# TAMUparametric/PPOPT

Hardware: NVIDIA B200
Metric: candidate active sets/sec (higher is better)
Workload: dtype f64

## Files before the change

### include/ppgpu.h

```cpp
#ifndef PPGPU_H
#define PPGPU_H

#include <stddef.h>
#include <stdint.h>

#ifdef __cplusplus
extern "C" {
#endif

typedef struct ppgpu_program ppgpu_program;
typedef void* ppgpu_stream;

typedef struct {
    int32_t n;
    int32_t t;
    int32_t m;
    int32_t q;
    int32_t n_eq;
    int32_t is_qp;
} ppgpu_dims;

typedef struct {
    int32_t words;
    int32_t n_ineq;
    int32_t region_rows;
    int32_t use_gram;
    int32_t max_depth;
    int32_t sm_count;
    int32_t lp_columns;
    int32_t reserved;
} ppgpu_info;

#define PPGPU_NUM_COUNTERS 24

const char* ppgpu_last_error(void);
int ppgpu_version(void);

int ppgpu_program_create(const ppgpu_dims* dims, const double* h_A, const double* h_b, const double* h_F,
                         const double* h_A_t, const double* h_b_t, const double* h_Q, const double* h_c,
                         const double* h_H, int device, ppgpu_program** out);
int ppgpu_program_destroy(ppgpu_program* prog);
int ppgpu_program_info(const ppgpu_program* prog, ppgpu_info* out);

#define PPGPU_OPT_K2W_MIN 0
int ppgpu_set_option(ppgpu_program* prog, int32_t option, int64_t value);

int ppgpu_root_level(ppgpu_program* prog, uint64_t* d_masks, int64_t* h_count, ppgpu_stream stream);

int ppgpu_level_eval(ppgpu_program* prog, const uint64_t* d_masks, int64_t n, int32_t k_act, uint8_t* d_status,
                     int32_t stages, ppgpu_stream stream);

#define PPGPU_WITNESS_SLOTS 2
int ppgpu_level_eval_w(ppgpu_program* prog, const uint64_t* d_masks, int64_t n, int32_t k_act, uint8_t* d_status,
                       int32_t stages, uint64_t* d_witness, const uint64_t* d_parent_feas, int64_t parent_nf,
                       const void* d_parent_ws, const uint64_t* d_parent_wit, ppgpu_stream stream);

size_t ppgpu_scan_workspace_bytes(int64_t n);
int ppgpu_level_select(ppgpu_program* prog, const uint8_t* d_status, int64_t n, uint8_t bits, uint8_t value,
                       int64_t* d_idx_out, int64_t* h_count, void* d_ws, size_t ws_bytes, ppgpu_stream stream);

int ppgpu_regions_emit(ppgpu_program* prog, const uint64_t* d_masks, const int64_t* d_sel, int64_t n_sel,
                       int32_t k_act, double* d_laws, double* d_rows, int32_t* d_flags, double* d_info,
                       uint8_t* d_status, ppgpu_stream stream);

int ppgpu_children_count(ppgpu_program* prog, const uint64_t* d_masks, const int64_t* d_feas_idx, int64_t nf,
                         int32_t k_act, uint64_t* d_feas_masks, uint64_t* d_survive, int64_t* d_offsets,
                         int64_t* h_total, void* d_ws, size_t ws_bytes, ppgpu_stream stream);
int ppgpu_children_prepare(ppgpu_program* prog, const uint64_t* d_masks, const int64_t* d_feas_idx, int64_t nf,
                           uint64_t* d_feas_masks, void* d_ws, size_t ws_bytes, ppgpu_stream stream);
int ppgpu_children_count_range(ppgpu_program* prog, const uint64_t* d_feas_masks, int64_t nf, int32_t k_act,
                               uint64_t* d_survive, int64_t* d_counts, int64_t p_lo, int64_t p_hi, void* d_ws,
                               size_t ws_bytes, ppgpu_stream stream);
int ppgpu_children_scan(ppgpu_program* prog, int64_t* d_counts_to_offsets, int64_t nf, int64_t* h_total, void* d_ws,
                        size_t ws_bytes, ppgpu_stream stream);
int ppgpu_children_write(ppgpu_program* prog, const uint64_t* d_feas_masks, const uint64_t* d_survive,
                         const int64_t* d_offsets, int64_t nf, uint64_t* d_children, ppgpu_stream stream);

int ppgpu_locate_points(const double* d_theta, int64_t n_points, int32_t t, const double* d_rows, const int64_t* d_row_off,
                        int64_t n_regions, const double* d_laws, int32_t n_x, int32_t use_tol, double tol, int32_t overlap,
                        const double* d_Q, const double* d_H, const double* d_c, int32_t* d_region, double* d_x,
                        ppgpu_stream stream);

int ppgpu_solve_theta_batch(ppgpu_program* prog, const double* d_theta, int64_t n_points, uint8_t* d_status, double* d_x,
                            double* d_dual, uint64_t* d_active, int32_t* d_iters, ppgpu_stream stream);

int ppgpu_solve_theta_lp_batch(ppgpu_program* prog, const double* d_theta, int64_t n_points, uint8_t* d_status, double* d_x,
                               double* d_dual, uint64_t* d_active, int32_t* d_iters, ppgpu_stream stream);

int ppgpu_chebyshev_batch(const double* d_rows, const int64_t* d_row_off, int64_t n_polytopes, int32_t t, int32_t max_rows,
                          double* d_radius, int32_t* d_code, ppgpu_stream stream);

int ppgpu_counters(ppgpu_program* prog, uint64_t* h_out, int32_t reset, ppgpu_stream stream);

int64_t ppgpu_launch_count(const ppgpu_program* prog);

#define PPGPU_NUM_FAMILIES 10
int ppgpu_profile_enable(ppgpu_program* prog, int32_t on);
int ppgpu_profile_read(ppgpu_program* prog, double* h_ms, int64_t* h_launches, int32_t reset);

int ppgpu_measure_fp64_peak(int32_t iters, double* h_tflops, ppgpu_stream stream);

#ifdef __cplusplus
}
#endif
#endif
```

### ppopt_b200/_lib.py

```python
import ctypes
import os

_HERE = os.path.dirname(os.path.abspath(__file__))
LIB_PATH = os.path.join(_HERE, 'libppgpu.so')

NUM_COUNTERS = 24
NUM_FAMILIES = 10
FAMILY_NAMES = ('k1_rank', 'k2_feas_lp', 'k34_kkt_cheb', 'k5_emit', 'k6_count', 'k6_write', 'select', 'k2a_relax', 'k2w_walk', 'inherit')
COUNTER_NAMES = ('k1_candidates', 'k2_lps', 'k2_pivots', 'k2_work', 'k4_lps', 'k4_pivots', 'k4_work', 'k5_lps',
                 'k5_pivots', 'k5_work', 'numeric', 'border', 'k6_lookups', 'k2a_tried', 'k2a_certified', 'k2a_steps', 'k2a_work',
                 'k2w_certified', 'k2w_pivots', 'k2w_work', 'k2w_giveup', 'inherited', 'inherit_lookups')

ST_RANK, ST_FEAS, ST_OPT, ST_REGION, ST_BORDER, ST_NUMERIC, ST_THIN = 1, 2, 4, 8, 16, 32, 64
OPT_K2W_MIN = 0
WITNESS_SLOTS = 2


class Dims(ctypes.Structure):
    _fields_ = [(k, ctypes.c_int32) for k in ('n', 't', 'm', 'q', 'n_eq', 'is_qp')]


class Info(ctypes.Structure):
    _fields_ = [(k, ctypes.c_int32) for k in
                ('words', 'n_ineq', 'region_rows', 'use_gram', 'max_depth', 'sm_count', 'lp_columns', 'reserved')]


_vp, _i32, _i64, _u8, _sz = ctypes.c_void_p, ctypes.c_int32, ctypes.c_int64, ctypes.c_uint8, ctypes.c_size_t
SYMBOLS = {
    'ppgpu_last_error': (ctypes.c_char_p, []),
    'ppgpu_version': (ctypes.c_int, []),
    'ppgpu_program_create': (ctypes.c_int, [ctypes.POINTER(Dims)] + [_vp] * 8 + [ctypes.c_int, ctypes.POINTER(_vp)]),
    'ppgpu_program_destroy': (ctypes.c_int, [_vp]),
    'ppgpu_program_info': (ctypes.c_int, [_vp, ctypes.POINTER(Info)]),
    'ppgpu_set_option': (ctypes.c_int, [_vp, _i32, _i64]),
    'ppgpu_root_level': (ctypes.c_int, [_vp, _vp, ctypes.POINTER(_i64), _vp]),
    'ppgpu_level_eval': (ctypes.c_int, [_vp, _vp, _i64, _i32, _vp, _i32, _vp]),
    'ppgpu_level_eval_w': (ctypes.c_int, [_vp, _vp, _i64, _i32, _vp, _i32, _vp, _vp, _i64, _vp, _vp, _vp]),
    'ppgpu_scan_workspace_bytes': (_sz, [_i64]),
    'ppgpu_level_select': (ctypes.c_int, [_vp, _vp, _i64, _u8, _u8, _vp, ctypes.POINTER(_i64), _vp, _sz, _vp]),
    'ppgpu_regions_emit': (ctypes.c_int, [_vp, _vp, _vp, _i64, _i32, _vp, _vp, _vp, _vp, _vp, _vp]),
    'ppgpu_children_count': (ctypes.c_int, [_vp, _vp, _vp, _i64, _i32, _vp, _vp, _vp, ctypes.POINTER(_i64), _vp, _sz, _vp]),
    'ppgpu_children_prepare': (ctypes.c_int, [_vp, _vp, _vp, _i64, _vp, _vp, _sz, _vp]),
    'ppgpu_children_count_range': (ctypes.c_int, [_vp, _vp, _i64, _i32, _vp, _vp, _i64, _i64, _vp, _sz, _vp]),
    'ppgpu_children_scan': (ctypes.c_int, [_vp, _vp, _i64, ctypes.POINTER(_i64), _vp, _sz, _vp]),
    'ppgpu_children_write': (ctypes.c_int, [_vp, _vp, _vp, _vp, _i64, _vp, _vp]),
    'ppgpu_counters': (ctypes.c_int, [_vp, _vp, _i32, _vp]),
    'ppgpu_launch_count': (_i64, [_vp]),
    'ppgpu_profile_enable': (ctypes.c_int, [_vp, _i32]),
    'ppgpu_profile_read': (ctypes.c_int, [_vp, _vp, _vp, _i32]),
    'ppgpu_locate_points': (ctypes.c_int, [_vp, _i64, _i32, _vp, _vp, _i64, _vp, _i32, _i32, ctypes.c_double, _i32, _vp, _vp, _vp,
                                           _vp, _vp, _vp]),
    'ppgpu_solve_theta_batch': (ctypes.c_int, [_vp, _vp, _i64, _vp, _vp, _vp, _vp, _vp, _vp]),
    'ppgpu_solve_theta_lp_batch': (ctypes.c_int, [_vp, _vp, _i64, _vp, _vp, _vp, _vp, _vp, _vp]),
    'ppgpu_chebyshev_batch': (ctypes.c_int, [_vp, _vp, _i64, _i32, _i32, _vp, _vp, _vp]),
    'ppgpu_measure_fp64_peak': (ctypes.c_int, [_i32, ctypes.POINTER(ctypes.c_double), _vp]),
}

_lib = None


def load():
    global _lib
    if _lib is not None:
        return _lib
    if not os.path.exists(LIB_PATH):
        raise RuntimeError(f'{LIB_PATH} is missing - build it with `make -C ppopt_b200/csrc` '
                           f'(or __graft_entry__.build()); ppopt_b200 has no CPU fallback')
    lib = ctypes.CDLL(LIB_PATH)
    for name, (res, args) in SYMBOLS.items():
        fn = getattr(lib, name)
        fn.restype = res
        fn.argtypes = args
    _lib = lib
    return lib


def check(rc, what=''):
    if rc != 0:
        msg = load().ppgpu_last_error()
        raise RuntimeError(f'libppgpu {what} failed ({rc}): {msg.decode() if msg else "?"}')
```

### ppopt_b200/csrc/api.cu

```cuda
#include <cstdio>
#include <cstdlib>
#include <cstring>
#include <mutex>
#include <string>
#include <vector>

#include "../../include/ppgpu.h"
#include "common.cuh"
#include "host_math.hpp"
#include "launch.h"

using namespace ppgpu;

static thread_local std::string g_err;

struct ppgpu_program {
    ReducedProgram host;
    DevProgram dev;
    int device = 0;
    int sm_count = 0;
    std::vector<void*> allocs;
    unsigned long long* d_counters = nullptr;
    unsigned long long* d_queue = nullptr;
    int queue_slot = 0;
    long long launches = 0;
    bool profiling = false;
    struct Span { int family; cudaEvent_t a, b; };
    std::vector<Span> spans;
    std::vector<cudaEvent_t> event_pool;
    long long warm_cap = 0;
    double* d_warm_resid = nullptr;
    long long* d_warm_idx = nullptr;
    unsigned long long* d_warm_count = nullptr;
    int* d_k2w_order = nullptr;
    size_t k2w_order_cap = 0;
    long long k2w_min = 100000;
    double prof_ms[PPGPU_NUM_FAMILIES] = {0};
    long long prof_launches[PPGPU_NUM_FAMILIES] = {0};
};

struct ProfScope {
    ppgpu_program* p; cudaStream_t st; int family; cudaEvent_t a = nullptr, b = nullptr;
    static cudaEvent_t get(ppgpu_program* p) {
        if (!p->event_pool.empty()) { cudaEvent_t e = p->event_pool.back(); p->event_pool.pop_back(); return e; }
        cudaEvent_t e; cudaEventCreate(&e); return e;
    }
    ProfScope(ppgpu_program* p_, cudaStream_t st_, int fam) : p(p_), st(st_), family(fam) {
        if (p->profiling) { a = get(p); b = get(p); cudaEventRecord(a, st); }
    }
    ~ProfScope() {
        if (a) { cudaEventRecord(b, st); p->spans.push_back({family, a, b}); }
    }
};

static const int QUEUE_SLOTS = 64;
extern "C" { static void warm_release(ppgpu_program* p); }

static int fail(const char* where, cudaError_t e) {
    g_err = std::string(where) + ": " + cudaGetErrorString(e);
    return -1;
}
static int fail_msg(const std::string& m) { g_err = m; return -2; }

template <class T>
static cudaError_t upload(ppgpu_program* p, const std::vector<T>& v, const T** out) {
    void* d = nullptr;
    const size_t bytes = v.size() * sizeof(T) + 1024;
    cudaError_t e = cudaMalloc(&d, bytes);
    if (e != cudaSuccess) return e;
    p->allocs.push_back(d);
    if ((e = cudaMemset(d, 0, bytes)) != cudaSuccess) return e;
    if (v.size()) e = cudaMemcpy(d, v.data(), v.size() * sizeof(T), cudaMemcpyHostToDevice);
    *out = (const T*)d;
    return e;
}

static unsigned long long* next_queue(ppgpu_program* p, cudaStream_t st) {
    unsigned long long* q = p->d_queue + p->queue_slot;
    p->queue_slot = (p->queue_slot + 1) % QUEUE_SLOTS;
    cudaMemsetAsync(q, 0, sizeof(unsigned long long), st);
    return q;
}

extern "C" {

const char* ppgpu_last_error(void) { return g_err.c_str(); }
int ppgpu_version(void) { return 100; }

int ppgpu_program_create(const ppgpu_dims* d, const double* A, const double* b, const double* F, const double* A_t,
                         const double* b_t, const double* Q, const double* c, const double* H, int device,
                         ppgpu_program** out) {
    if (!d || !out) return fail_msg("null argument");
    if (d->is_qp && !Q) return fail_msg("is_qp set but Q is NULL");
    ppgpu_program* p = new ppgpu_program();
    if (!reduce_program(d->n, d->t, d->m, d->q, d->n_eq, d->is_qp, A, b, F, A_t, b_t, Q, c, H, p->host)) {
        std::string m = "program reduction failed: " + p->host.error;
        delete p;
        return fail_msg(m);
    }
    const ReducedProgram& R = p->host;
    if (R.W > 4) { delete p; return fail_msg("more than 256 inequality rows are not supported"); }
    if (R.R0 > 256) { delete p; return fail_msg("more than 256 region rows ((m - n_eq) + q) are not supported"); }
    if (k2_pad_columns(R.nfree + 2) < 0) { delete p; return fail_msg("n - n_eq + t + 2 > 64 columns are not supported"); }
    if (R.t + 2 > 16) { delete p; return fail_msg("more than 14 parameters are not supported"); }
    if (R.np > 64) { delete p; return fail_msg("n - n_eq > 64 is not supported"); }
    {
        const int depth = (R.n > R.t ? R.n : R.t) - R.ne, k = R.ne + (depth > 0 ? depth : 0), N = R.n + k, ld = N + R.t + 1;
        const size_t smem = ((size_t)N * ld + (size_t)R.R0 * (R.t + 1)) * sizeof(double) + (size_t)(2 * R.R0 + k + 2) * sizeof(int);
        if (smem > 200 * 1024) {
            delete p;
            return fail_msg("region emission needs " + std::to_string(smem / 1024) + " KB of shared memory at the deepest level (n + k = " +
                            std::to_string(N) + "); the limit is 200 KB (about n + k <= 150)");
        }
    }
    cudaError_t e = cudaSetDevice(device);
    if (e != cudaSuccess) { delete p; return fail("cudaSetDevice", e); }
    p->device = device;
    cudaDeviceGetAttribute(&p->sm_count, cudaDevAttrMultiProcessorCount, device);
    DevProgram& D = p->dev;
    D.n = R.n; D.t = R.t; D.m = R.m; D.q = R.q; D.ne = R.ne; D.is_qp = R.is_qp;
    D.mi = R.mi; D.np = R.np; D.W = R.W; D.R0 = R.R0; D.nfree = R.nfree; D.use_gram = R.use_gram;
    D.dc0 = R.nfree + 2;
#define UP(field, vecname) if ((e = upload(p, R.vecname, &D.field)) != cudaSuccess) { ppgpu_program_destroy(p); return fail("upload " #field, e); }
    UP(At, At) UP(C1, C1) UP(T0, T0) UP(Gam, Gam) UP(G, G) UP(V, V) UP(th_lo, th_lo) UP(th_hi, th_hi) UP(A, A) UP(b, b) UP(F, F) UP(A_t, At_theta) UP(b_t, bt) UP(Q, Q) UP(c, c) UP(H, H)
    UP(Xp, Xp) UP(K, K) UP(Pm, Pm)
#undef UP
    D.wk_ok = R.wk_ok; D.wk_nb = R.wk_nb; D.wk_ld = R.wk_ld; D.wk_D0 = nullptr; D.wk_bvar = nullptr; D.wk_nvar = nullptr;
    if (R.wk_ok) {
        if ((e = upload(p, R.wk_D0, &D.wk_D0)) != cudaSuccess || (e = upload(p, R.wk_bvar, &D.wk_bvar)) != cudaSuccess ||
            (e = upload(p, R.wk_nvar, &D.wk_nvar)) != cudaSuccess) { ppgpu_program_destroy(p); return fail("upload walk dictionary", e); }
    }
    D.lp_ok = R.lp_ok; D.lp_ld = R.lp_ld; D.lp_D0 = nullptr; D.lp_bvar = nullptr; D.lp_nvar = nullptr; D.lp_obj = nullptr;
    D.X0t = nullptr; D.Q2 = nullptr;
    if (R.lp_ok) {
        if ((e = upload(p, R.lp_D0, &D.lp_D0)) != cudaSuccess || (e = upload(p, R.lp_bvar, &D.lp_bvar)) != cudaSuccess ||
            (e = upload(p, R.lp_nvar, &D.lp_nvar)) != cudaSuccess || (e = upload(p, R.lp_obj, &D.lp_obj)) != cudaSuccess ||
            (e = upload(p, R.X0t, &D.X0t)) != cudaSuccess || (e = upload(p, R.Q2, &D.Q2)) != cudaSuccess) {
            ppgpu_program_destroy(p);
            return fail("upload LP start dictionary", e);
        }
    }
    void* dc = nullptr;
    if ((e = cudaMalloc(&dc, (CNT_COUNT + QUEUE_SLOTS) * sizeof(unsigned long long))) != cudaSuccess) {
        ppgpu_program_destroy(p);
        return fail("cudaMalloc counters", e);
    }
    p->allocs.push_back(dc);
    cudaMemset(dc, 0, (CNT_COUNT + QUEUE_SLOTS) * sizeof(unsigned long long));
    p->d_counters = (unsigned long long*)dc;
    p->d_queue = p->d_counters + CNT_COUNT;
    *out = p;
    return 0;
}

int ppgpu_program_destroy(ppgpu_program* p) {
    if (!p) return 0;
    for (void* d : p->allocs) cudaFree(d);
    if (p->d_k2w_order) cudaFree(p->d_k2w_order);
    warm_release(p);
    for (auto& s : p->spans) { cudaEventDestroy(s.a); cudaEventDestroy(s.b); }
    for (cudaEvent_t e : p->event_pool) cudaEventDestroy(e);
    delete p;
    return 0;
}

int ppgpu_set_option(ppgpu_program* p, int32_t option, int64_t value) {
    if (!p) return fail_msg("null argument");
    switch (option) {
        case PPGPU_OPT_K2W_MIN: p->k2w_min = value; return 0;
        default: return fail_msg("unknown option");
    }
}

int ppgpu_program_info(const ppgpu_program* p, ppgpu_info* o) {
    if (!p || !o) return fail_msg("null argument");
    const ReducedProgram& R = p->host;
    o->words = R.W; o->n_ineq = R.mi; o->region_rows = R.R0; o->use_gram = R.use_gram;
    o->max_depth = (R.n > R.t ? R.n : R.t) - R.ne;
    o->sm_count = p->sm_count;
    o->lp_columns = k2_pad_columns(R.nfree + 2);
    o->reserved = R.wk_ok;
    return 0;
}

int ppgpu_root_level(ppgpu_program* p, uint64_t* d_masks, int64_t* h_count, ppgpu_stream stream) {
    if (!p || !h_count) return fail_msg("null argument");
    long long cnt = 0;
    cudaError_t e = root_level(p->dev, d_masks, &cnt, (cudaStream_t)stream);
    if (e != cudaSuccess) return fail("root_level", e);
    p->launches += cnt > 0;
    *h_count = cnt;
    return 0;
}

static long long level_chunk() {
    static const long long c = getenv("PPGPU_CHUNK") ? atoll(getenv("PPGPU_CHUNK")) : (1ll << 22);
    return c < 1024 ? 1024 : c;
}
static long long walk_chunk() {
    static const long long c = getenv("PPGPU_WALK_CHUNK") ? atoll(getenv("PPGPU_WALK_CHUNK")) : (1ll << 27);
    return c < 1024 ? 1024 : c;
}

struct WarmBuf { int device; size_t resid_bytes, idx_bytes; double* resid; long long* idx; };
static std::mutex g_pool_mu;
static std::vector<WarmBuf> g_pool;

static void warm_release(ppgpu_program* p) {
    if (!p->d_warm_resid) return;
    std::lock_guard<std::mutex> lk(g_pool_mu);
    if (g_pool.size() < 4) {
        g_pool.push_back({p->device, (size_t)p->warm_cap * p->dev.R0 * sizeof(double),
                          (size_t)p->warm_cap * sizeof(long long), p->d_warm_resid, p->d_warm_idx});
    } else {
        cudaFree(p->d_warm_resid);
        cudaFree(p->d_warm_idx);
    }
    p->d_warm_resid = nullptr; p->d_warm_idx = nullptr; p->warm_cap = 0;
}

static cudaError_t ensure_warm(ppgpu_program* p, long long cap, cudaStream_t st) {
    if (!p->d_warm_count) {
        cudaError_t e = cudaMalloc((void**)&p->d_warm_count, sizeof(unsigned long long));
        if (e != cudaSuccess) return e;
        p->allocs.push_back(p->d_warm_count);
    }
    if (cap <= p->warm_cap) return cudaSuccess;
    const long long full = 4096 + level_chunk() / 8;
    const long long want = cap <= 65536 ? 65536 : (cap > full ? cap : full);
    cudaError_t e = cudaStreamSynchronize(st);
    if (e != cudaSuccess) return e;
    warm_release(p);
    const size_t rb = (size_t)want * p->dev.R0 * sizeof(double), ib = (size_t)want * sizeof(long long);
    {
        std::lock_guard<std::mutex> lk(g_pool_mu);
        for (size_t i = 0; i < g_pool.size(); ++i) {
            if (g_pool[i].device == p->device && g_pool[i].resid_bytes >= rb && g_pool[i].idx_bytes >= ib) {
                p->d_warm_resid = g_pool[i].resid; p->d_warm_idx = g_pool[i].idx; p->warm_cap = want;
                g_pool.erase(g_pool.begin() + i);
                return cudaSuccess;
            }
        }
    }
    if ((e = cudaMalloc((void**)&p->d_warm_resid, rb)) != cudaSuccess) return e;
    if ((e = cudaMalloc((void**)&p->d_warm_idx, ib)) != cudaSuccess) { cudaFree(p->d_warm_resid); p->d_warm_resid = nullptr; return e; }
    p->warm_cap = want;
    return cudaSuccess;
}

static_assert(PPGPU_WITNESS_SLOTS == PPG_WITNESS_SLOTS, "witness slots: include/ppgpu.h and csrc/tolerances.h disagree");
struct WitnessIo {
    uint64_t* out = nullptr;
    const uint64_t* parent_feas = nullptr;
    long long parent_nf = 0;
    const void* parent_ws = nullptr;
    const uint64_t* parent_wit = nullptr;
};

static int level_eval_chunk(ppgpu_program* p, const uint64_t* d_masks, int64_t n, int32_t k_act, uint8_t* d_status,
                            int32_t stages, cudaStream_t st, const WitnessIo& wio) {
    cudaError_t e;
    if (stages & 1) {
        ProfScope ps(p, st, 0);
        const long long piece = 1ll << 22;
        for (long long off = 0; off < n; off += piece) {
            const long long nn = n - off < piece ? n - off : piece;
            e = launch_k1(p->dev, d_masks + (size_t)off * p->dev.W, nn, k_act, d_status + off, p->d_counters, p->sm_count, st);
            if (e != cudaSuccess) return fail("K1 rank", e);
            if (k_act >= 1 && k_act <= 8) p->launches++;
            p->launches++;
            if (k_act >= 2 && k_act <= p->dev.np) p->launches++;
        }
    }
    if ((stages & 2) && !(stages & 8) && wio.parent_feas && wio.parent_wit && wio.parent_ws && wio.parent_nf > 0) {
        ProfScope ps(p, st, 9);
        e = launch_inherit(p->dev, d_masks, n, d_status, wio.out, wio.parent_feas, wio.parent_nf, wio.parent_ws,
                           wio.parent_wit, p->d_counters, st);
        if (e != cudaSuccess) return fail("witness inheritance", e);
        p->launches++;
    }
    static const int warm_on = getenv("PPGPU_WARM") ? atoi(getenv("PPGPU_WARM")) : 1;
    p->dev.warm_count = nullptr; p->dev.warm_resid = nullptr; p->dev.warm_idx = nullptr; p->dev.warm_cap = 0;
    if ((stages & 2) && !(stages & 8) && k_act >= 1 && p->k2w_min >= 0 && n >= p->k2w_min) {
        ProfScope ps(p, st, 8);
        bool handled = false;
        const size_t want = k2w_order_scratch_ints(walk_chunk());
        if (want > p->k2w_order_cap) {
            if ((e = cudaStreamSynchronize(st)) != cudaSuccess) return fail("K2w order scratch", e);
            if (p->d_k2w_order) cudaFree(p->d_k2w_order);
            p->d_k2w_order = nullptr; p->k2w_order_cap = 0;
            if ((e = cudaMalloc((void**)&p->d_k2w_order, want * sizeof(int))) != cudaSuccess) return fail("K2w order scratch", e);
            p->k2w_order_cap = want;
        }
        e = launch_k2w(p->dev, d_masks, n, k_act, d_status, next_queue(p, st), p->d_counters, p->sm_count, st, &handled, wio.out, p->d_k2w_order);
        if (e != cudaSuccess) return fail("K2w vertex walk", e);
        if (handled) p->launches += (n > 128ll * 8 * p->sm_count) ? 4 : 1;
    }
    if ((stages & 2) && !(stages & 8)) {
        ProfScope ps(p, st, 7);
        static const int iters = getenv("PPGPU_K2A_ITERS") ? atoi(getenv("PPGPU_K2A_ITERS")) : 96;
        if (iters > 0 && k_act >= 0) {
            if (warm_on) {
                const bool walked = k_act >= 1 && p->dev.wk_ok && p->k2w_min >= 0 && n >= p->k2w_min;
                const long long cap = n < 4096 ? n : 4096 + n / (walked ? 64 : 8);
                if ((e = ensure_warm(p, cap, st)) != cudaSuccess) return fail("warm-start buffers", e);
                p->dev.warm_count = p->d_warm_count; p->dev.warm_resid = p->d_warm_resid;
                p->dev.warm_idx = p->d_warm_idx; p->dev.warm_cap = cap;
                cudaMemsetAsync(p->d_warm_count, 0, sizeof(unsigned long long), st);
            }
            e = launch_k2a(p->dev, d_masks, n, k_act, d_status, next_queue(p, st), p->d_counters, iters,
                           p->sm_count, st);
            if (e != cudaSuccess) return fail("K2a relaxation", e);
            p->launches++;
        }
    }
    if (stages & 2) {
        ProfScope ps(p, st, 1);
        e = launch_k2(p->dev, d_masks, n, d_status, next_queue(p, st), p->d_counters, p->sm_count, st);
        if (e != cudaSuccess) return fail("K2 feasibility", e);
        p->launches++;
        if (p->dev.warm_count) {
            if ((e = launch_clear_bits(d_status, n, PPG_ST_PRE, st)) != cudaSuccess) return fail("status clean-up", e);
            p->launches++;
        }
    }
    if (stages & 4) {
        ProfScope ps(p, st, 2);
        if (p->dev.is_qp && p->dev.use_gram) {
            e = launch_k34(p->dev, d_masks, n, k_act, d_status, next_queue(p, st), p->d_counters, p->sm_count, st);
            if (k_act >= 1 && k_act <= 8) p->launches++;
        } else {
            e = launch_mark_general(p->dev, n, k_act, d_status, st);
        }
        if (e != cudaSuccess) return fail("K3/K4 optimality screen", e);
        p->launches++;
    }
    return 0;
}

int ppgpu_level_eval(ppgpu_program* p, const uint64_t* d_masks, int64_t n, int32_t k_act, uint8_t* d_status,
                     int32_t stages, ppgpu_stream stream) {
    return ppgpu_level_eval_w(p, d_masks, n, k_act, d_status, stages, nullptr, nullptr, 0, nullptr, nullptr, stream);
}

int ppgpu_level_eval_w(ppgpu_program* p, const uint64_t* d_masks, int64_t n, int32_t k_act, uint8_t* d_status,
                       int32_t stages, uint64_t* d_witness, const uint64_t* d_parent_feas, int64_t parent_nf,
                       const void* d_parent_ws, const uint64_t* d_parent_wit, ppgpu_stream stream) {
    if (!p) return fail_msg("null argument");
    if (n <= 0) return 0;
    WitnessIo wio;
    wio.parent_feas = d_parent_feas; wio.parent_nf = parent_nf; wio.parent_ws = d_parent_ws; wio.parent_wit = d_parent_wit;
    const bool walk = (stages & 2) && !(stages & 8) && k_act >= 1 && p->dev.wk_ok && p->k2w_min >= 0 && n >= p->k2w_min;
    const long long chunk = walk ? walk_chunk() : level_chunk();
    for (int64_t off = 0; off < n; off += chunk) {
        const int64_t nn = n - off < chunk ? n - off : chunk;
        wio.out = d_witness ? d_witness + (size_t)off * PPGPU_WITNESS_SLOTS * p->dev.W : nullptr;
        const int rc = level_eval_chunk(p, d_masks + (size_t)off * p->dev.W, nn, k_act, d_status + off, stages,
                                        (cudaStream_t)stream, wio);
        if (rc) return rc;
    }
    return 0;
}

size_t ppgpu_scan_workspace_bytes(int64_t n) { return scan_workspace_bytes(n); }

int ppgpu_level_select(ppgpu_program* p, const uint8_t* d_status, int64_t n, uint8_t bits, uint8_t value,
                       int64_t* d_idx_out, int64_t* h_count, void* d_ws, size_t ws_bytes, ppgpu_stream stream) {
    if (!p || !h_count) return fail_msg("null argument");
    *h_count = 0;
    if (n <= 0) return 0;
    cudaStream_t st = (cudaStream_t)stream;
    if (ws_bytes < scan_workspace_bytes(n)) return fail_msg("workspace too small");
    long long* d_count = (long long*)d_ws + (scan_workspace_bytes(n) / sizeof(long long) - 1);
    cudaError_t e;
    {
        ProfScope ps(p, st, 6);
        e = select_indices(d_status, n, bits, value, (long long*)d_idx_out, d_count, d_ws, ws_bytes - sizeof(long long), st);
    }
    if (e != cudaSuccess) return fail("select", e);
    p->launches += 5;
    long long cnt = 0;
    e = cudaMemcpyAsync(&cnt, d_count, sizeof(long long), cudaMemcpyDeviceToHost, st);
    if (e == cudaSuccess) e = cudaStreamSynchronize(st);
    if (e != cudaSuccess) return fail("select count", e);
    *h_count = cnt;
    return 0;
}

int ppgpu_regions_emit(ppgpu_program* p, const uint64_t* d_masks, const int64_t* d_sel, int64_t n_sel, int32_t k_act,
                       double* d_laws, double* d_rows, int32_t* d_flags, double* d_info, uint8_t* d_status,
                       ppgpu_stream stream) {
    if (!p) return fail_msg("null argument");
    if (n_sel <= 0) return 0;
    cudaError_t e;
    {
        ProfScope ps(p, (cudaStream_t)stream, 3);
        e = launch_k5(p->dev, d_masks, (const long long*)d_sel, n_sel, k_act, d_laws, d_rows, d_flags, d_info, d_status,
                      p->d_counters, p->sm_count, (cudaStream_t)stream);
    }
    if (e != cudaSuccess) return fail("K5 emit", e);
    p->launches++;
    return 0;
}

int ppgpu_children_count(ppgpu_program* p, const uint64_t* d_masks, const int64_t* d_feas_idx, int64_t nf,
                         int32_t k_act, uint64_t* d_feas_masks, uint64_t* d_survive, int64_t* d_offsets,
                         int64_t* h_total, void* d_ws, size_t ws_bytes, ppgpu_stream stream) {
    if (!p || !h_total) return fail_msg("null argument");
    *h_total = 0;
    if (nf <= 0) return 0;
    cudaStream_t st = (cudaStream_t)stream;
    cudaError_t e;
    {
        ProfScope ps(p, st, 4);
        e = children_count(p->dev, d_masks, (const long long*)d_feas_idx, nf, k_act, d_feas_masks, d_survive,
                           (long long*)d_offsets, d_ws, ws_bytes, p->d_counters, st);
    }
    if (e != cudaSuccess) return fail("K6 count", e);
    p->launches += 5;
    long long tot = 0;
    e = cudaMemcpyAsync(&tot, (long long*)d_offsets + nf, sizeof(long long), cudaMemcpyDeviceToHost, st);
    if (e == cudaSuccess) e = cudaStreamSynchronize(st);
    if (e != cudaSuccess) return fail("K6 total", e);
    *h_total = tot;
    return 0;
}

int ppgpu_children_prepare(ppgpu_program* p, const uint64_t* d_masks, const int64_t* d_feas_idx, int64_t nf,
                           uint64_t* d_feas_masks, void* d_ws, size_t ws_bytes, ppgpu_stream stream) {
    if (!p) return fail_msg("null argument");
    if (nf <= 0) return 0;
    cudaError_t e;
    {
        ProfScope ps(p, (cudaStream_t)stream, 4);
        e = children_prepare(p->dev, d_masks, (const long long*)d_feas_idx, nf, d_feas_masks, d_ws, ws_bytes, (cudaStream_t)stream);
    }
    if (e != cudaSuccess) return fail("K6 prepare", e);
    p->launches += 3;
    return 0;
}

int ppgpu_children_count_range(ppgpu_program* p, const uint64_t* d_feas_masks, int64_t nf, int32_t k_act,
                               uint64_t* d_survive, int64_t* d_counts, int64_t p_lo, int64_t p_hi, void* d_ws,
                               size_t ws_bytes, ppgpu_stream stream) {
    if (!p) return fail_msg("null argument");
    if (p_lo < 0 || p_hi > nf || p_lo > p_hi) return fail_msg("parent range outside [0, nf]");
    if (nf <= 0 || p_hi == p_lo) return 0;
    if (ws_bytes < scan_workspace_bytes(nf)) return fail_msg("workspace too small");
    cudaError_t e;
    {
        ProfScope ps(p, (cudaStream_t)stream, 4);
        e = children_count_range(p->dev, d_feas_masks, nf, k_act, d_survive, (long long*)d_counts, p_lo, p_hi, d_ws,
                                 p->d_counters, (cudaStream_t)stream);
    }
    if (e != cudaSuccess) return fail("K6 count", e);
    p->launches++;
    return 0;
}

int ppgpu_children_scan(ppgpu_program* p, int64_t* d_counts_to_offsets, int64_t nf, int64_t* h_total, void* d_ws,
                        size_t ws_bytes, ppgpu_stream stream) {
    if (!p || !h_total) return fail_msg("null argument");
    *h_total = 0;
    if (nf <= 0) return 0;
    if (ws_bytes < scan_workspace_bytes(nf)) return fail_msg("workspace too small");
    cudaStream_t st = (cudaStream_t)stream;
    cudaError_t e;
    {
        ProfScope ps(p, st, 4);
        e = children_scan((long long*)d_counts_to_offsets, nf, d_ws, st);
    }
    if (e != cudaSuccess) return fail("K6 scan", e);
    p->launches += 2;
    long long tot = 0;
    e = cudaMemcpyAsync(&tot, (long long*)d_counts_to_offsets + nf, sizeof(long long), cudaMemcpyDeviceToHost, st);
    if (e == cudaSuccess) e = cudaStreamSynchronize(st);
    if (e != cudaSuccess) return fail("K6 total", e);
    *h_total = tot;
    return 0;
}

int ppgpu_children_write(ppgpu_program* p, const uint64_t* d_feas_masks, const uint64_t* d_survive,
                         const int64_t* d_offsets, int64_t nf, uint64_t* d_children, ppgpu_stream stream) {
    if (!p) return fail_msg("null argument");
    cudaError_t e;
    {
        ProfScope ps(p, (cudaStream_t)stream, 5);
        e = children_write(p->dev, d_feas_masks, d_survive, (const long long*)d_offsets, nf, d_children, (cudaStream_t)stream);
    }
    if (e != cudaSuccess) return fail("K6 write", e);
    p->launches += nf > 0;
    return 0;
}

int ppgpu_counters(ppgpu_program* p, uint64_t* h_out, int32_t reset, ppgpu_stream stream) {
    if (!p || !h_out) return fail_msg("null argument");
    cudaStream_t st = (cudaStream_t)stream;
    cudaError_t e = cudaMemcpyAsync(h_out, p->d_counters, CNT_COUNT * sizeof(unsigned long long), cudaMemcpyDeviceToHost, st);
    if (e == cudaSuccess) e = cudaStreamSynchronize(st);
    if (e == cudaSuccess && reset) e = cudaMemsetAsync(p->d_counters, 0, CNT_COUNT * sizeof(unsigned long long), st);
    if (e != cudaSuccess) return fail("counters", e);
    return 0;
}

int64_t ppgpu_launch_count(const ppgpu_program* p) { return p ? p->launches : 0; }

int ppgpu_profile_enable(ppgpu_program* p, int32_t on) {
    if (!p) return fail_msg("null argument");
    p->profiling = on != 0;
    return 0;
}

int ppgpu_profile_read(ppgpu_program* p, double* h_ms, int64_t* h_launches, int32_t reset) {
    if (!p || !h_ms || !h_launches) return fail_msg("null argument");
    for (auto& s : p->spans) {
        cudaError_t e = cudaEventSynchronize(s.b);
        if (e != cudaSuccess) return fail("profile sync", e);
        float ms = 0.f;
        cudaEventElapsedTime(&ms, s.a, s.b);
        p->prof_ms[s.family] += ms;
        p->prof_launches[s.family] += 1;
        p->event_pool.push_back(s.a);
        p->event_pool.push_back(s.b);
    }
    p->spans.clear();
    for (int f = 0; f < PPGPU_NUM_FAMILIES; ++f) { h_ms[f] = p->prof_ms[f]; h_launches[f] = p->prof_launches[f]; }
    if (reset) for (int f = 0; f < PPGPU_NUM_FAMILIES; ++f) { p->prof_ms[f] = 0; p->prof_launches[f] = 0; }
    return 0;
}

int ppgpu_locate_points(const double* d_theta, int64_t n_points, int32_t t, const double* d_rows, const int64_t* d_row_off,
                        int64_t n_regions, const double* d_laws, int32_t n_x, int32_t use_tol, double tol, int32_t overlap,
                        const double* d_Q, const double* d_H, const double* d_c, int32_t* d_region, double* d_x,
                        ppgpu_stream stream) {
    if (n_points < 0 || n_regions < 0 || n_x < 0) return fail_msg("negative size");
    if (n_points == 0) return 0;
    if (!d_theta || !d_region || !d_row_off || (n_regions > 0 && !d_rows)) return fail_msg("null argument");
    if ((d_x || overlap) && n_x > 0 && n_regions > 0 && !d_laws) return fail_msg("laws needed (d_x or overlap) but d_laws is NULL");
    if (t < 1 || t > 32) return fail_msg("point location supports 1 <= t <= 32 parameters");
    if (overlap && (n_x < 1 || n_x > 128)) return fail_msg("the overlapping rule supports 1 <= n_x <= 128 variables");
    if (overlap && (!d_H || !d_c)) return fail_msg("the overlapping rule needs the objective (d_H, d_c; d_Q for an mpQP)");
    int dev = 0, sms = 0;
    cudaError_t e = cudaGetDevice(&dev);
    if (e == cudaSuccess) e = cudaDeviceGetAttribute(&sms, cudaDevAttrMultiProcessorCount, dev);
    if (e != cudaSuccess) return fail("device query", e);
    e = launch_locate(d_theta, n_points, t, d_rows, (const long long*)d_row_off, n_regions, d_laws, n_x, use_tol, tol,
                      overlap ? 1 : 0, d_Q, d_H, d_c, d_region, d_x, sms, (cudaStream_t)stream);
    if (e != cudaSuccess) return fail("K7 point location", e);
    return 0;
}

int ppgpu_solve_theta_batch(ppgpu_program* p, const double* d_theta, int64_t n_points, uint8_t* d_status, double* d_x,
                            double* d_dual, uint64_t* d_active, int32_t* d_iters, ppgpu_stream stream) {
    if (!p) return fail_msg("null argument");
    if (!p->dev.is_qp || !p->dev.use_gram)
        return fail_msg("solve_theta needs an mpQP whose Hessian is positive definite on the reduced space (use_gram = 0)");
    if (n_points < 0) return fail_msg("negative size");
    if (n_points == 0) return 0;
    if (!d_theta || !d_status) return fail_msg("null argument");
    cudaError_t e = cudaSetDevice(p->device);
    if (e == cudaSuccess)
        e = launch_theta_qp(p->dev, d_theta, n_points, d_status, d_x, d_dual, d_active, d_iters, p->sm_count, (cudaStream_t)stream);
    if (e != cudaSuccess) return fail("K8 fixed-theta QP", e);
    p->launches++;
    return 0;
}

int ppgpu_solve_theta_lp_batch(ppgpu_program* p, const double* d_theta, int64_t n_points, uint8_t* d_status, double* d_x,
                               double* d_dual, uint64_t* d_active, int32_t* d_iters, ppgpu_stream stream) {
    if (!p) return fail_msg("null argument");
    if (p->dev.is_qp) return fail_msg("solve_theta_lp needs an mpLP handle (this one is an mpQP: ppgpu_solve_theta_batch)");
    if (!p->dev.lp_ok) return fail_msg("solve_theta_lp: the reduced inequality rows have rank below n - n_eq, the LP has no vertex");
    if (n_points < 0) return fail_msg("negative size");
    if (n_points == 0) return 0;
    if (!d_theta || !d_status) return fail_msg("null argument");
    cudaError_t e = cudaSetDevice(p->device);
    if (e == cudaSuccess)
        e = launch_theta_lp(p->dev, d_theta, n_points, d_status, d_x, d_dual, d_active, d_iters, p->sm_count, (cudaStream_t)stream);
    if (e != cudaSuccess) return fail("K9 fixed-theta LP", e);
    p->launches++;
    return 0;
}

int ppgpu_chebyshev_batch(const double* d_rows, const int64_t* d_row_off, int64_t n_polytopes, int32_t t, int32_t max_rows,
                          double* d_radius, int32_t* d_code, ppgpu_stream stream) {
    if (n_polytopes < 0) return fail_msg("negative size");
    if (n_polytopes == 0) return 0;
    if (!d_rows || !d_row_off || !d_radius || !d_code) return fail_msg("null argument");
    if (t < 1 || t > 30) return fail_msg("the Chebyshev batch supports 1 <= t <= 30 parameters");
    if (max_rows < 1 || max_rows > 1024) return fail_msg("the Chebyshev batch supports 1..1024 rows per polytope");
    int dev = 0, sms = 0;
    cudaError_t e = cudaGetDevice(&dev);
    if (e == cudaSuccess) e = cudaDeviceGetAttribute(&sms, cudaDevAttrMultiProcessorCount, dev);
    if (e != cudaSuccess) return fail("device query", e);
    e = launch_cheb_batch(d_rows, (const long long*)d_row_off, n_polytopes, t, max_rows, d_radius, d_code, sms, (cudaStream_t)stream);
    if (e != cudaSuccess) return fail("Chebyshev batch", e);
    return 0;
}

int ppgpu_measure_fp64_peak(int32_t iters, double* h_tflops, ppgpu_stream stream) {
    if (!h_tflops) return fail_msg("null argument");
    cudaError_t e = measure_fp64_peak(iters, h_tflops, (cudaStream_t)stream);
    if (e != cudaSuccess) return fail("fp64 peak", e);
    return 0;
}

}
```

### ppopt_b200/csrc/k6_children.cu

```cuda
#include "common.cuh"
#include "launch.h"

namespace ppgpu {

constexpr int SCAN_THREADS = 256;
constexpr int SCAN_ITEMS = 8;
constexpr int SCAN_CHUNK = SCAN_THREADS * SCAN_ITEMS;

__device__ __forceinline__ long long block_exclusive_scan(long long v, long long* total) {
    __shared__ long long wsum[SCAN_THREADS / 32];
    const int lane = threadIdx.x & 31, warp = threadIdx.x >> 5;
    long long x = v;
#pragma unroll
    for (int o = 1; o < 32; o <<= 1) {
        const long long y = __shfl_up_sync(0xffffffffu, x, o);
        if (lane >= o) x += y;
    }
    if (lane == 31) wsum[warp] = x;
    __syncthreads();
    long long wpre = 0, tot = 0;
#pragma unroll
    for (int w = 0; w < SCAN_THREADS / 32; ++w) {
        if (w < warp) wpre += wsum[w];
        tot += wsum[w];
    }
    __syncthreads();
    *total = tot;
    return wpre + x - v;
}

__global__ void __launch_bounds__(SCAN_THREADS) scan_block_sums_kernel(const long long* __restrict__ in, long long n,
                                                                        long long* __restrict__ bsum) {
    const long long base = (long long)blockIdx.x * SCAN_CHUNK;
    long long s = 0;
#pragma unroll
    for (int k = 0; k < SCAN_ITEMS; ++k) {
        const long long i = base + (long long)k * SCAN_THREADS + threadIdx.x;
        if (i < n) s += in[i];
    }
    long long tot;
    block_exclusive_scan(s, &tot);
    if (threadIdx.x == 0) bsum[blockIdx.x] = tot;
}

__global__ void __launch_bounds__(SCAN_THREADS) scan_bsums_kernel(long long* __restrict__ bsum, long long nb) {
    __shared__ long long carry_s;
    if (threadIdx.x == 0) carry_s = 0;
    __syncthreads();
    for (long long base = 0; base < nb; base += SCAN_THREADS) {
        const long long i = base + threadIdx.x;
        const long long v = i < nb ? bsum[i] : 0;
        long long tot;
        const long long ex = block_exclusive_scan(v, &tot);
        const long long carry = carry_s;
        if (i < nb) bsum[i] = carry + ex;
        __syncthreads();
        if (threadIdx.x == 0) carry_s = carry + tot;
        __syncthreads();
    }
    if (threadIdx.x == 0) bsum[nb] = carry_s;
}

__global__ void __launch_bounds__(SCAN_THREADS) scan_apply_kernel(const long long* in, long long n,
                                                                   const long long* __restrict__ bsum, long long nb,
                                                                   long long* out) {
    const long long base = (long long)blockIdx.x * SCAN_CHUNK + (long long)threadIdx.x * SCAN_ITEMS;
    long long v[SCAN_ITEMS];
    long long s = 0;
#pragma unroll
    for (int k = 0; k < SCAN_ITEMS; ++k) {
        const long long i = base + k;
        v[k] = i < n ? in[i] : 0;
        s += v[k];
    }
    long long tot;
    long long ex = block_exclusive_scan(s, &tot) + bsum[blockIdx.x];
#pragma unroll
    for (int k = 0; k < SCAN_ITEMS; ++k) {
        const long long i = base + k;
        if (i < n) out[i] = ex;
        ex += v[k];
    }
    if (blockIdx.x == 0 && threadIdx.x == 0) out[n] = bsum[nb];
}


size_t scan_workspace_bytes(long long n) {
    const long long nb = (n + SCAN_CHUNK - 1) / SCAN_CHUNK + 1;
    const long long table = 2 * n + 2 > 1024 ? 2 * n + 2 : 1024;
    return (size_t)(n + 1 + nb + 2 + table) * sizeof(long long);
}

static cudaError_t scan_inplace(long long* vals, long long n, long long* bsum, cudaStream_t st) {
    const long long nb = (n + SCAN_CHUNK - 1) / SCAN_CHUNK;
    if (n == 0) return cudaMemsetAsync(vals, 0, sizeof(long long), st);
    scan_block_sums_kernel<<<(unsigned)nb, SCAN_THREADS, 0, st>>>(vals, n, bsum);
    scan_bsums_kernel<<<1, SCAN_THREADS, 0, st>>>(bsum, nb);
    scan_apply_kernel<<<(unsigned)nb, SCAN_THREADS, 0, st>>>(vals, n, bsum, nb, vals);
    return cudaGetLastError();
}

__global__ void select_flag_kernel(const uint8_t* __restrict__ status, long long n, uint8_t bits, uint8_t value,
                                   long long* __restrict__ flag) {
    const long long i = (long long)blockIdx.x * blockDim.x + threadIdx.x;
    if (i < n) flag[i] = ((status[i] & bits) == value) ? 1 : 0;
}

__global__ void select_scatter_kernel(const uint8_t* __restrict__ status, long long n, uint8_t bits, uint8_t value,
                                      const long long* __restrict__ offs, long long* __restrict__ idx_out) {
    const long long i = (long long)blockIdx.x * blockDim.x + threadIdx.x;
    if (i < n && ((status[i] & bits) == value)) idx_out[offs[i]] = i;
}

cudaError_t select_indices(const uint8_t* status, long long n, uint8_t bits, uint8_t value, long long* idx_out,
                           long long* d_count, void* ws, size_t ws_bytes, cudaStream_t st) {
    if (ws_bytes + sizeof(long long) < (size_t)(n + 1 + (n + SCAN_CHUNK - 1) / SCAN_CHUNK + 3) * sizeof(long long)) return cudaErrorInvalidValue;
    long long* offs = (long long*)ws;
    long long* bsum = offs + n + 1;
    if (n == 0) return cudaMemsetAsync(d_count, 0, sizeof(long long), st);
    const unsigned blocks = (unsigned)((n + 255) / 256);
    select_flag_kernel<<<blocks, 256, 0, st>>>(status, n, bits, value, offs);
    cudaError_t e = scan_inplace(offs, n, bsum, st);
    if (e != cudaSuccess) return e;
    select_scatter_kernel<<<blocks, 256, 0, st>>>(status, n, bits, value, offs, idx_out);
    return cudaMemcpyAsync(d_count, offs + n, sizeof(long long), cudaMemcpyDeviceToDevice, st);
}

__global__ void root_level_kernel(int W, long long count, uint64_t* __restrict__ masks) {
    const long long i = (long long)blockIdx.x * blockDim.x + threadIdx.x;
    if (i < count) {
        for (int w = 0; w < W; ++w) masks[i * W + w] = 0ull;
        masks[i * W + (i >> 6)] = 1ull << (i & 63);
    }
}

cudaError_t root_level(const DevProgram& P, uint64_t* masks, long long* h_count, cudaStream_t st) {
    long long count = P.mi;
    if (!P.is_qp) {
        long long lim = (long long)1 + P.m - P.n;
        if (lim < 0) lim = 0;
        if (count > lim) count = lim;
    }
    *h_count = count;
    if (count == 0) return cudaSuccess;
    root_level_kernel<<<(unsigned)((count + 255) / 256), 256, 0, st>>>(P.W, count, masks);
    return cudaGetLastError();
}

constexpr int MAXW = 4;

__global__ void gather_masks_kernel(const uint64_t* __restrict__ masks, const long long* __restrict__ idx, long long nf, int W,
                                    uint64_t* __restrict__ out) {
    const long long e = (long long)blockIdx.x * blockDim.x + threadIdx.x;
    if (e < nf * W) {
        const long long p = e / W;
        const int w = (int)(e - p * W);
        out[e] = masks[idx[p] * W + w];
    }
}

struct Mask4 { uint64_t w[MAXW]; };

__device__ __forceinline__ int lex_cmp4(const uint64_t* __restrict__ a, const Mask4& b, int W) {
    int res = 0;
#pragma unroll
    for (int x = 0; x < MAXW; ++x) {
        if (x < W && res == 0) {
            const uint64_t av = a[x];
            const uint64_t d = av ^ b.w[x];
            if (d) {
                const uint64_t low = d & (~d + 1ull);
                res = (av & low) ? -1 : 1;
            }
        }
    }
    return res;
}

__device__ __forceinline__ unsigned hash_mask(const Mask4& k, int W) {
    uint64_t h = 0x9e3779b97f4a7c15ull;
#pragma unroll
    for (int x = 0; x < MAXW; ++x)
        if (x < W) { h ^= k.w[x]; h *= 0xff51afd7ed558ccdull; h ^= h >> 32; }
    return (unsigned)h;
}

__global__ void hash_insert_kernel(const uint64_t* __restrict__ feas, long long nf, int W, int* __restrict__ table, unsigned cap_mask) {
    const long long p = (long long)blockIdx.x * blockDim.x + threadIdx.x;
    if (p >= nf) return;
    Mask4 k;
#pragma unroll
    for (int x = 0; x < MAXW; ++x) k.w[x] = x < W ? feas[p * W + x] : 0ull;
    unsigned slot = hash_mask(k, W) & cap_mask;
    while (atomicCAS(&table[slot], -1, (int)p) != -1) slot = (slot + 1) & cap_mask;
}

__device__ __forceinline__ bool hash_contains(const uint64_t* __restrict__ feas, int W, const int* __restrict__ table,
                                              unsigned cap_mask, const Mask4& key) {
    unsigned slot = hash_mask(key, W) & cap_mask;
    for (;;) {
        const int e = __ldg(table + slot);
        if (e < 0) return false;
        bool same = true;
#pragma unroll
        for (int x = 0; x < MAXW; ++x)
            if (x < W && feas[(long long)e * W + x] != key.w[x]) same = false;
        if (same) return true;
        slot = (slot + 1) & cap_mask;
    }
}

__global__ void __launch_bounds__(128)
children_count_kernel(DevProgram P, const uint64_t* __restrict__ feas, long long p_lo, long long p_hi, int k_act,
                      uint64_t* __restrict__ survive, long long* __restrict__ counts,
                      unsigned long long* __restrict__ counters, const int* __restrict__ table, unsigned cap_mask) {
    const int lane = threadIdx.x & 31;
    const long long warp0 = ((long long)blockIdx.x * blockDim.x + threadIdx.x) >> 5;
    const long long nwarps = ((long long)gridDim.x * blockDim.x) >> 5;
    const int W = P.W, mi = P.mi;
    const bool lp = !P.is_qp;
    const int child_limit = lp ? (P.ne + k_act + 1) + P.m - P.n : 0x7fffffff;
    const int sub_limit = lp ? (P.ne + k_act) + P.m - P.n : 0x7fffffff;
    unsigned long long lookups = 0;
    for (long long p = p_lo + warp0; p < p_hi; p += nwarps) {
        uint64_t pm[MAXW];
#pragma unroll
        for (int w = 0; w < MAXW; ++w) pm[w] = w < W ? feas[p * W + w] : 0ull;
        int last = -1;
#pragma unroll
        for (int w = MAXW - 1; w >= 0; --w)
            if (last < 0 && pm[w]) last = w * 64 + 63 - __clzll((long long)pm[w]);
        long long cnt = 0;
        uint64_t sv[MAXW];
#pragma unroll
        for (int w = 0; w < MAXW; ++w) sv[w] = 0ull;
        for (int base = ((last + 1) >> 5) << 5; base < mi; base += 32) {
            const int i = base + lane;
            bool ok = i > last && i < mi && (P.ne + i) < child_limit;
            if (ok) {
                const bool sub_filtered = (P.ne + i) >= sub_limit;
                if (!sub_filtered) {
                    Mask4 child;
#pragma unroll
                    for (int w = 0; w < MAXW; ++w) child.w[w] = pm[w] | ((w == (i >> 6)) ? (1ull << (i & 63)) : 0ull);
#pragma unroll
                    for (int w = 0; w < MAXW; ++w) {
                        if (w < W) {
                            uint64_t bits = pm[w];
                            while (bits && ok) {
                                const int b = __ffsll((long long)bits) - 1;
                                bits &= bits - 1;
                                Mask4 sub;
#pragma unroll
                                for (int x = 0; x < MAXW; ++x) sub.w[x] = child.w[x] & ~((x == w) ? (1ull << b) : 0ull);
                                ++lookups;
                                if (!hash_contains(feas, W, table, cap_mask, sub)) ok = false;
                            }
                        }
                    }
                }
            }
            const unsigned bal = __ballot_sync(0xffffffffu, ok);
            cnt += __popc(bal);
#pragma unroll
            for (int w = 0; w < MAXW; ++w)
                if (w == (base >> 6)) sv[w] |= (uint64_t)bal << (base & 63);
        }
        if (lane == 0) {
            counts[p] = cnt;
            for (int w = 0; w < W; ++w) survive[p * W + w] = sv[w];
        }
    }
#pragma unroll
    for (int o = 16; o > 0; o >>= 1) lookups += __shfl_xor_sync(0xffffffffu, lookups, o);
    if (lane == 0 && lookups) atomicAdd(&counters[CNT_K6_LOOKUPS], lookups);
}

__global__ void __launch_bounds__(128)
children_write_kernel(int W, const uint64_t* __restrict__ feas, const uint64_t* __restrict__ survive,
                      const long long* __restrict__ offsets, long long nf, uint64_t* __restrict__ children) {
    const int lane = threadIdx.x & 31;
    const long long warp0 = ((long long)blockIdx.x * blockDim.x + threadIdx.x) >> 5;
    const long long nwarps = ((long long)gridDim.x * blockDim.x) >> 5;
    for (long long p = warp0; p < nf; p += nwarps) {
        long long off = offsets[p];
        for (int w = 0; w < W; ++w) {
            const uint64_t x = survive[p * W + w];
            const int tot = __popcll(x);
            for (int r = lane; r < tot; r += 32) {
                const int b = mask_nth(&x, 1, r);
                uint64_t* dst = children + (off + r) * W;
                for (int y = 0; y < W; ++y) dst[y] = feas[p * W + y] | (y == w ? (1ull << b) : 0ull);
            }
            off += tot;
        }
    }
}

static unsigned hash_capacity(long long nf) {
    unsigned cap = 1024;
    while ((long long)cap < 2 * nf) cap <<= 1;
    return cap;
}

cudaError_t children_prepare(const DevProgram& P, const uint64_t* masks, const long long* feas_idx, long long nf,
                             uint64_t* feas_masks, void* ws, size_t ws_bytes, cudaStream_t st) {
    if (P.W > MAXW) return cudaErrorInvalidValue;
    if (nf <= 0) return cudaSuccess;
    if (nf >= (1ll << 30)) return cudaErrorInvalidValue;
    const long long nb = (nf + SCAN_CHUNK - 1) / SCAN_CHUNK;
    const unsigned cap = hash_capacity(nf);
    if (ws_bytes < (size_t)(nb + 2) * sizeof(long long) + (size_t)cap * sizeof(int)) return cudaErrorInvalidValue;
    int* table = reinterpret_cast<int*>((long long*)ws + nb + 2);
    const long long ne = nf * P.W;
    gather_masks_kernel<<<(unsigned)((ne + 255) / 256), 256, 0, st>>>(masks, feas_idx, nf, P.W, feas_masks);
    cudaError_t e = cudaMemsetAsync(table, 0xff, (size_t)cap * sizeof(int), st);
    if (e != cudaSuccess) return e;
    hash_insert_kernel<<<(unsigned)((nf + 255) / 256), 256, 0, st>>>(feas_masks, nf, P.W, table, cap - 1);
    return cudaGetLastError();
}

cudaError_t children_count_range(const DevProgram& P, const uint64_t* feas_masks, long long nf, int k_act, uint64_t* survive,
                                 long long* counts, long long p_lo, long long p_hi, void* ws, unsigned long long* counters,
                                 cudaStream_t st) {
    if (p_hi <= p_lo) return cudaSuccess;
    const long long nb = (nf + SCAN_CHUNK - 1) / SCAN_CHUNK;
    const unsigned cap = hash_capacity(nf);
    const int* table = reinterpret_cast<const int*>((long long*)ws + nb + 2);
    long long blocks = ((p_hi - p_lo) * 32 + 127) / 128;
    if (blocks > 148 * 64) blocks = 148 * 64;
    children_count_kernel<<<(unsigned)blocks, 128, 0, st>>>(P, feas_masks, p_lo, p_hi, k_act, survive, counts, counters, table,
                                                            cap - 1);
    return cudaGetLastError();
}

cudaError_t children_scan(long long* counts_to_offsets, long long nf, void* ws, cudaStream_t st) {
    if (nf == 0) return cudaMemsetAsync(counts_to_offsets, 0, sizeof(long long), st);
    return scan_inplace(counts_to_offsets, nf, (long long*)ws, st);
}

cudaError_t children_count(const DevProgram& P, const uint64_t* masks, const long long* feas_idx, long long nf, int k_act,
                           uint64_t* feas_masks, uint64_t* survive, long long* offsets, void* ws, size_t ws_bytes,
                           unsigned long long* counters, cudaStream_t st) {
    if (nf == 0) return cudaMemsetAsync(offsets, 0, sizeof(long long), st);
    cudaError_t e = children_prepare(P, masks, feas_idx, nf, feas_masks, ws, ws_bytes, st);
    if (e != cudaSuccess) return e;
    if ((e = children_count_range(P, feas_masks, nf, k_act, survive, offsets, 0, nf, ws, counters, st)) != cudaSuccess) return e;
    return children_scan(offsets, nf, ws, st);
}

cudaError_t children_write(const DevProgram& P, const uint64_t* feas_masks, const uint64_t* survive, const long long* offsets,
                           long long nf, uint64_t* children, cudaStream_t st) {
    if (nf == 0) return cudaSuccess;
    long long blocks = (nf * 32 + 127) / 128;
    if (blocks > 148 * 64) blocks = 148 * 64;
    children_write_kernel<<<(unsigned)blocks, 128, 0, st>>>(P.W, feas_masks, survive, offsets, nf, children);
    return cudaGetLastError();
}

__device__ __forceinline__ int hash_find(const uint64_t* __restrict__ feas, int W, const int* __restrict__ table,
                                         unsigned cap_mask, const Mask4& key) {
    unsigned slot = hash_mask(key, W) & cap_mask;
    for (;;) {
        const int e = __ldg(table + slot);
        if (e < 0) return -1;
        bool same = true;
#pragma unroll
        for (int x = 0; x < MAXW; ++x)
            if (x < W && feas[(long long)e * W + x] != key.w[x]) same = false;
        if (same) return e;
        slot = (slot + 1) & cap_mask;
    }
}

__global__ void __launch_bounds__(256)
inherit_kernel(int W, const uint64_t* __restrict__ masks, long long n, uint8_t* __restrict__ status,
               uint64_t* __restrict__ witness_out, const uint64_t* __restrict__ pfeas, const int* __restrict__ table,
               unsigned cap_mask, const uint64_t* __restrict__ pwit, unsigned long long* __restrict__ counters) {
    const long long i = (long long)blockIdx.x * blockDim.x + threadIdx.x;
    unsigned long long lookups = 0;
    int got = 0;
    if (i < n) {
        const uint8_t sb = status[i];
        if ((sb & PPG_ST_RANK) && !(sb & PPG_ST_FEAS)) {
            Mask4 m;
#pragma unroll
            for (int x = 0; x < MAXW; ++x) m.w[x] = x < W ? masks[i * W + x] : 0ull;
#pragma unroll
            for (int w = MAXW - 1; w >= 0; --w) {
                if (w < W && !got) {
                    uint64_t bits = m.w[w];
                    while (bits && !got) {
                        const int b = 63 - __clzll((long long)bits);
                        bits &= ~(1ull << b);
                        Mask4 sub = m;
#pragma unroll
                        for (int x = 0; x < MAXW; ++x)
                            if (x == w) sub.w[x] &= ~(1ull << b);
                        ++lookups;
                        const int e = hash_find(pfeas, W, table, cap_mask, sub);
                        if (e < 0) continue;
#pragma unroll
                        for (int sl = 0; sl < PPG_WITNESS_SLOTS; ++sl) {
                            if (got) continue;
                            bool inside = true;
                            uint64_t wv[MAXW];
#pragma unroll
                            for (int x = 0; x < MAXW; ++x) {
                                wv[x] = x < W ? __ldg(pwit + ((long long)e * PPG_WITNESS_SLOTS + sl) * W + x) : 0ull;
                                if (m.w[x] & ~wv[x]) inside = false;
                            }
                            if (inside) {
                                got = 1;
                                status[i] = sb | PPG_ST_FEAS;
                                if (witness_out)
#pragma unroll
                                    for (int x = 0; x < MAXW; ++x)
                                        if (x < W) witness_out[i * (PPG_WITNESS_SLOTS * W) + x] = wv[x];
                            }
                        }
                    }
                }
            }
        }
    }
    got = __reduce_add_sync(0xffffffffu, got);
#pragma unroll
    for (int o = 16; o > 0; o >>= 1) lookups += __shfl_xor_sync(0xffffffffu, lookups, o);
    if ((threadIdx.x & 31) == 0 && lookups) {
        atomicAdd(&counters[CNT_INHERITED], (unsigned long long)got);
        atomicAdd(&counters[CNT_INHERIT_LOOKUPS], lookups);
    }
}

cudaError_t launch_inherit(const DevProgram& P, const uint64_t* masks, long long n, uint8_t* status, uint64_t* witness_out,
                           const uint64_t* parent_feas, long long parent_nf, const void* parent_ws, const uint64_t* parent_wit,
                           unsigned long long* counters, cudaStream_t st) {
    if (n <= 0 || parent_nf <= 0) return cudaSuccess;
    if (P.W > MAXW) return cudaErrorInvalidValue;
    const long long nb = (parent_nf + SCAN_CHUNK - 1) / SCAN_CHUNK;
    const unsigned cap = hash_capacity(parent_nf);
    const int* table = reinterpret_cast<const int*>((const long long*)parent_ws + nb + 2);
    inherit_kernel<<<(unsigned)((n + 255) / 256), 256, 0, st>>>(P.W, masks, n, status, witness_out, parent_feas, table, cap - 1,
                                                                parent_wit, counters);
    return cudaGetLastError();
}

__global__ void __launch_bounds__(256) dfma_peak_kernel(int iters, double* sink) {
    double a0 = threadIdx.x * 1e-3, a1 = a0 + 1, a2 = a0 + 2, a3 = a0 + 3, a4 = a0 + 4, a5 = a0 + 5, a6 = a0 + 6, a7 = a0 + 7;
    const double m = 0.999999, c = 1e-9;
    for (int i = 0; i < iters; ++i) {
        a0 = fma(a0, m, c); a1 = fma(a1, m, c); a2 = fma(a2, m, c); a3 = fma(a3, m, c);
        a4 = fma(a4, m, c); a5 = fma(a5, m, c); a6 = fma(a6, m, c); a7 = fma(a7, m, c);
    }
    const double s = a0 + a1 + a2 + a3 + a4 + a5 + a6 + a7;
    if (s == 123.456) sink[0] = s;
}

cudaError_t measure_fp64_peak(int iters, double* tflops, cudaStream_t st) {
    int dev = 0, sms = 0;
    cudaGetDevice(&dev);
    cudaDeviceGetAttribute(&sms, cudaDevAttrMultiProcessorCount, dev);
    double* sink = nullptr;
    cudaError_t e = cudaMalloc(&sink, sizeof(double));
    if (e != cudaSuccess) return e;
    cudaEvent_t a, b;
    cudaEventCreate(&a); cudaEventCreate(&b);
    const int blocks = sms * 8;
    dfma_peak_kernel<<<blocks, 256, 0, st>>>(iters / 10 + 1, sink);
    float best = 1e30f;
    for (int rep = 0; rep < 3; ++rep) {
        cudaEventRecord(a, st);
        dfma_peak_kernel<<<blocks, 256, 0, st>>>(iters, sink);
        cudaEventRecord(b, st);
        cudaEventSynchronize(b);
        float ms = 0;
        cudaEventElapsedTime(&ms, a, b);
        if (ms < best) best = ms;
    }
    cudaEventDestroy(a); cudaEventDestroy(b);
    cudaFree(sink);
    e = cudaGetLastError();
    const double flops = 2.0 * 8.0 * (double)iters * 256.0 * blocks;
    *tflops = flops / (best * 1e-3) / 1e12;
    return e;
}

}
```

### ppopt_b200/csrc/launch.h

```cpp
#pragma once
#include <cuda_runtime.h>
#include <stdint.h>

#include "common.cuh"

namespace ppgpu {

template <class K>
inline cudaError_t allow_max_smem(K kern) {
    int dev = 0, lim = 0;
    cudaError_t e = cudaGetDevice(&dev);
    if (e == cudaSuccess) e = cudaDeviceGetAttribute(&lim, cudaDevAttrMaxSharedMemoryPerBlockOptin, dev);
    if (e != cudaSuccess) return e;
    cudaFuncAttributes fa;
    if ((e = cudaFuncGetAttributes(&fa, kern)) != cudaSuccess) return e;
    return cudaFuncSetAttribute(kern, cudaFuncAttributeMaxDynamicSharedMemorySize, lim - (int)fa.sharedSizeBytes);
}

template <class K>
inline cudaError_t fit_smem(K kern, size_t dyn) {
    cudaFuncAttributes fa;
    const cudaError_t e = cudaFuncGetAttributes(&fa, kern);
    if (e != cudaSuccess) return e;
    return fa.sharedSizeBytes + dyn > 48 * 1024 ? allow_max_smem(kern) : cudaSuccess;
}

int k2_pad_columns(int ncols_with_rhs);

cudaError_t launch_k1(const DevProgram& P, const uint64_t* masks, long long n, int k_act, uint8_t* status,
                      unsigned long long* counters, int sm_count, cudaStream_t st);
cudaError_t launch_k2(const DevProgram& P, const uint64_t* masks, long long n, uint8_t* status,
                      unsigned long long* queue, unsigned long long* counters, int sm_count, cudaStream_t st);
cudaError_t launch_k2a(const DevProgram& P, const uint64_t* masks, long long n, int k_act, uint8_t* status,
                       unsigned long long* queue, unsigned long long* counters, int max_iter, int sm_count, cudaStream_t st);
cudaError_t launch_k2a_prefix(const DevProgram& P, const uint64_t* masks, long long n, int k_act, uint8_t* status,
                              unsigned long long* queue, unsigned long long* counters, int max_iter, int sm_count,
                              cudaStream_t st, bool* handled);
cudaError_t launch_k2w(const DevProgram& P, const uint64_t* masks, long long n, int k_act, uint8_t* status,
                       unsigned long long* queue, unsigned long long* counters, int sm_count, cudaStream_t st, bool* handled,
                       uint64_t* witness, int* order_scratch);
size_t k2w_order_scratch_ints(long long n);
cudaError_t launch_inherit(const DevProgram& P, const uint64_t* masks, long long n, uint8_t* status, uint64_t* witness_out,
                           const uint64_t* parent_feas, long long parent_nf, const void* parent_ws, const uint64_t* parent_wit,
                           unsigned long long* counters, cudaStream_t st);
cudaError_t launch_k34(const DevProgram& P, const uint64_t* masks, long long n, int k_act, uint8_t* status,
                       unsigned long long* queue, unsigned long long* counters, int sm_count, cudaStream_t st);
cudaError_t launch_k34_compact(const DevProgram& P, const uint64_t* masks, long long n, int k_act, uint8_t* status,
                               unsigned long long* queue, unsigned long long* counters, int sm_count, cudaStream_t st,
                               int use_pre, bool* handled);
cudaError_t launch_mark_general(const DevProgram& P, long long n, int k_act, uint8_t* status, cudaStream_t st);

cudaError_t launch_k5(const DevProgram& P, const uint64_t* masks, const long long* idx, long long n_sel, int k_act,
                      double* laws, double* rows, int32_t* flags, double* info, uint8_t* status,
                      unsigned long long* counters, int sm_count, cudaStream_t st);

size_t scan_workspace_bytes(long long n);
cudaError_t select_indices(const uint8_t* status, long long n, uint8_t bits, uint8_t value, long long* idx_out,
                           long long* d_count, void* ws, size_t ws_bytes, cudaStream_t st);
cudaError_t root_level(const DevProgram& P, uint64_t* masks, long long* d_count, cudaStream_t st);
cudaError_t children_count(const DevProgram& P, const uint64_t* masks, const long long* feas_idx, long long nf,
                           int k_act, uint64_t* feas_masks, uint64_t* survive, long long* offsets, void* ws,
                           size_t ws_bytes, unsigned long long* counters, cudaStream_t st);
cudaError_t children_prepare(const DevProgram& P, const uint64_t* masks, const long long* feas_idx, long long nf,
                             uint64_t* feas_masks, void* ws, size_t ws_bytes, cudaStream_t st);
cudaError_t children_count_range(const DevProgram& P, const uint64_t* feas_masks, long long nf, int k_act, uint64_t* survive,
                                 long long* counts, long long p_lo, long long p_hi, void* ws, unsigned long long* counters,
                                 cudaStream_t st);
cudaError_t children_scan(long long* counts_to_offsets, long long nf, void* ws, cudaStream_t st);
cudaError_t children_write(const DevProgram& P, const uint64_t* feas_masks, const uint64_t* survive,
                           const long long* offsets, long long nf, uint64_t* children, cudaStream_t st);

cudaError_t launch_locate(const double* theta, long long n_points, int t, const double* rows, const long long* row_off,
                          long long n_regions, const double* laws, int n_x, int use_tol, double tol, int overlap,
                          const double* Qm, const double* Hm, const double* cv, int* region_out, double* x_out, int sm_count,
                          cudaStream_t st);

cudaError_t launch_cheb_batch(const double* rows, const long long* row_off, long long n_poly, int t, int max_rows,
                              double* radius, int* code, int sm_count, cudaStream_t st);
cudaError_t launch_theta_qp(const DevProgram& P, const double* theta, long long n_points, uint8_t* status, double* x,
                            double* dual, uint64_t* mask, int* iters, int sm_count, cudaStream_t st);
cudaError_t launch_theta_lp(const DevProgram& P, const double* theta, long long n_points, uint8_t* status, double* x,
                            double* dual, uint64_t* mask, int* iters, int sm_count, cudaStream_t st);
cudaError_t launch_clear_bits(uint8_t* status, long long n, uint8_t bits, cudaStream_t st);

cudaError_t measure_fp64_peak(int iters, double* tflops, cudaStream_t st);

}
```

### ppopt_b200/engine.py

```python
import ctypes
import time
from typing import Dict, List, Optional

import numpy
import torch

from . import _lib, sharding
from ._lib import ST_BORDER, ST_FEAS, ST_NUMERIC, ST_OPT, ST_RANK, ST_REGION, ST_THIN


def _c(a):
    return numpy.ascontiguousarray(numpy.asarray(a, dtype=numpy.float64))


def program_arrays(program) -> Dict:
    A = _c(program.A)
    n = A.shape[1]
    F = _c(program.F)
    t = F.shape[1]
    is_qp = hasattr(program, 'Q') and program.Q is not None and type(program).__name__ != 'MPLP_Program'
    H = _c(program.H)
    if H.shape != (n, t):
        if H.shape == (t, n) and not numpy.any(H):
            H = numpy.zeros((n, t))
        else:
            raise ValueError(f'H must be num_x x num_t = {(n, t)}, got {H.shape}')
    eq = [int(i) for i in program.equality_indices]
    if eq != list(range(len(eq))):
        raise ValueError('equality_indices must be range(n_eq) (the reference constructor guarantees it)')
    out = dict(A=A, b=_c(program.b).reshape(-1), F=F, A_t=_c(program.A_t).reshape(-1, t),
               b_t=_c(program.b_t).reshape(-1), c=_c(program.c).reshape(-1), H=H, n_eq=len(eq), is_qp=bool(is_qp))
    out['Q'] = _c(program.Q) if is_qp else None
    return out


class Engine:

    def __init__(self, arrays: Dict, device: Optional[int] = None):
        if not torch.cuda.is_available():
            raise RuntimeError('ppopt_b200 needs a CUDA device (there is no CPU fallback)')
        self.lib = _lib.load()
        self.device = torch.cuda.current_device() if device is None else int(device)
        self.tdev = torch.device('cuda', self.device)
        a = arrays
        self.n, self.t = a['A'].shape[1], a['F'].shape[1]
        self.m, self.q, self.n_eq, self.is_qp = a['A'].shape[0], a['A_t'].shape[0], a['n_eq'], a['is_qp']
        dims = _lib.Dims(self.n, self.t, self.m, self.q, self.n_eq, int(self.is_qp))
        self._keep = a
        h = ctypes.c_void_p()
        ptr = lambda x: None if x is None else x.ctypes.data
        with torch.cuda.device(self.device):
            rc = self.lib.ppgpu_program_create(ctypes.byref(dims), ptr(a['A']), ptr(a['b']), ptr(a['F']), ptr(a['A_t']),
                                               ptr(a['b_t']), ptr(a['Q']), ptr(a['c']), ptr(a['H']), self.device,
                                               ctypes.byref(h))
        _lib.check(rc, 'program_create')
        self.h = h
        info = _lib.Info()
        _lib.check(self.lib.ppgpu_program_info(self.h, ctypes.byref(info)), 'program_info')
        self.W, self.mi, self.R0 = info.words, info.n_ineq, info.region_rows
        self.use_gram, self.max_depth, self.sm_count = bool(info.use_gram), info.max_depth, info.sm_count
        self.lp_columns = info.lp_columns
        self.has_walk_vertex = bool(info.reserved)
        self.h2d_bytes = sum(v.nbytes for v in a.values() if isinstance(v, numpy.ndarray))
        self.d2h_bytes = 0

    def close(self):
        if getattr(self, 'h', None) is not None and self.h:
            self.lib.ppgpu_program_destroy(self.h)
            self.h = None

    def __del__(self):
        try:
            self.close()
        except Exception:
            pass

    def set_option(self, option: int, value: int):
        _lib.check(self.lib.ppgpu_set_option(self.h, int(option), int(value)), 'set_option')

    def _stream(self):
        return ctypes.c_void_p(torch.cuda.current_stream(self.tdev).cuda_stream)

    def empty(self, shape, dtype):
        return torch.empty(shape, dtype=dtype, device=self.tdev)

    def root_level(self) -> torch.Tensor:
        masks = self.empty((max(self.mi, 1), self.W), torch.int64)
        cnt = ctypes.c_int64(0)
        _lib.check(self.lib.ppgpu_root_level(self.h, masks.data_ptr(), ctypes.byref(cnt), self._stream()), 'root_level')
        return masks[:cnt.value]

    def level_eval(self, masks: torch.Tensor, k_act: int, status: Optional[torch.Tensor] = None, stages: int = 7,
                   lo: int = 0, hi: Optional[int] = None, witness: Optional[torch.Tensor] = None,
                   parent: Optional['ParentLevel'] = None) -> torch.Tensor:
        n = masks.shape[0]
        if status is None:
            status = torch.zeros((n,), dtype=torch.uint8, device=self.tdev)
        hi = n if hi is None else hi
        if hi > lo:
            if witness is None and parent is None:
                _lib.check(self.lib.ppgpu_level_eval(self.h, masks.data_ptr() + lo * self.W * 8, hi - lo, k_act,
                                                     status.data_ptr() + lo, stages, self._stream()), 'level_eval')
            else:
                pf, pnf, pws, pw = (parent.feas_masks.data_ptr(), parent.nf, parent.ws.data_ptr(), parent.wit.data_ptr()) \
                    if parent is not None else (None, 0, None, None)
                _lib.check(self.lib.ppgpu_level_eval_w(self.h, masks.data_ptr() + lo * self.W * 8, hi - lo, k_act,
                                                       status.data_ptr() + lo, stages,
                                                       None if witness is None else witness.data_ptr() + lo * _lib.WITNESS_SLOTS * self.W * 8,
                                                       pf, pnf, pws, pw, self._stream()), 'level_eval_w')
        return status

    def select(self, status: torch.Tensor, bits: int, value: int) -> torch.Tensor:
        n = status.shape[0]
        if n == 0:
            return self.empty((0,), torch.int64)
        ws_bytes = self.lib.ppgpu_scan_workspace_bytes(n)
        ws = self.empty(((ws_bytes + 7) // 8,), torch.int64)
        idx = self.empty((n,), torch.int64)
        cnt = ctypes.c_int64(0)
        _lib.check(self.lib.ppgpu_level_select(self.h, status.data_ptr(), n, bits, value, idx.data_ptr(), ctypes.byref(cnt),
                                               ws.data_ptr(), ws_bytes, self._stream()), 'level_select')
        return idx[:cnt.value]

    def emit(self, masks: torch.Tensor, sel: torch.Tensor, k_act: int, status: torch.Tensor):
        ns = sel.shape[0]
        N = self.n + self.n_eq + k_act
        laws = self.empty((ns, N, self.t + 1), torch.float64)
        rows = self.empty((ns, self.R0, self.t + 1), torch.float64)
        flags = self.empty((ns, self.R0), torch.int32)
        info = self.empty((ns, 4), torch.float64)
        _lib.check(self.lib.ppgpu_regions_emit(self.h, masks.data_ptr(), sel.data_ptr(), ns, k_act, laws.data_ptr(),
                                               rows.data_ptr(), flags.data_ptr(), info.data_ptr(), status.data_ptr(),
                                               self._stream()), 'regions_emit')
        return laws, rows, flags, info

    def children(self, masks: torch.Tensor, feas_idx: torch.Tensor, k_act: int, dist=None, keep: Optional[dict] = None) -> torch.Tensor:
        nf = feas_idx.shape[0]
        if nf == 0:
            return self.empty((0, self.W), torch.int64)
        if dist is not None and dist.get_world_size() > 1 and nf >= 65536:
            return self._children_sharded(masks, feas_idx, k_act, dist, keep)
        feas_masks = self.empty((nf, self.W), torch.int64)
        survive = self.empty((nf, self.W), torch.int64)
        offsets = self.empty((nf + 1,), torch.int64)
        ws_bytes = self.lib.ppgpu_scan_workspace_bytes(nf)
        ws = self.empty(((ws_bytes + 7) // 8,), torch.int64)
        tot = ctypes.c_int64(0)
        _lib.check(self.lib.ppgpu_children_count(self.h, masks.data_ptr(), feas_idx.data_ptr(), nf, k_act,
                                                 feas_masks.data_ptr(), survive.data_ptr(), offsets.data_ptr(),
                                                 ctypes.byref(tot), ws.data_ptr(), ws_bytes, self._stream()),
                   'children_count')
        if keep is not None:
            keep.update(feas_masks=feas_masks, ws=ws, nf=nf)
        out = self.empty((tot.value, self.W), torch.int64)
        if tot.value:
            _lib.check(self.lib.ppgpu_children_write(self.h, feas_masks.data_ptr(), survive.data_ptr(), offsets.data_ptr(),
                                                     nf, out.data_ptr(), self._stream()), 'children_write')
        return out

    def _children_sharded(self, masks, feas_idx, k_act, dist, keep=None):
        from . import sharding
        nf = feas_idx.shape[0]
        feas_masks = self.empty((nf, self.W), torch.int64)
        survive = torch.zeros((nf, self.W), dtype=torch.int64, device=self.tdev)
        counts = torch.zeros((nf + 1,), dtype=torch.int64, device=self.tdev)
        ws_bytes = self.lib.ppgpu_scan_workspace_bytes(nf)
        ws = self.empty(((ws_bytes + 7) // 8,), torch.int64)
        _lib.check(self.lib.ppgpu_children_prepare(self.h, masks.data_ptr(), feas_idx.data_ptr(), nf, feas_masks.data_ptr(),
                                                   ws.data_ptr(), ws_bytes, self._stream()), 'children_prepare')
        if keep is not None:
            keep.update(feas_masks=feas_masks, ws=ws, nf=nf)
        for lo, hi in sharding.chunks(nf, dist.get_rank(), dist.get_world_size()):
            _lib.check(self.lib.ppgpu_children_count_range(self.h, feas_masks.data_ptr(), nf, k_act, survive.data_ptr(),
                                                           counts.data_ptr(), lo, hi, ws.data_ptr(), ws_bytes,
                                                           self._stream()), 'children_count_range')
        dist.all_reduce(survive, op=dist.ReduceOp.SUM)
        dist.all_reduce(counts, op=dist.ReduceOp.SUM)
        tot = ctypes.c_int64(0)
        _lib.check(self.lib.ppgpu_children_scan(self.h, counts.data_ptr(), nf, ctypes.byref(tot), ws.data_ptr(), ws_bytes,
                                                self._stream()), 'children_scan')
        out = self.empty((tot.value, self.W), torch.int64)
        if tot.value:
            _lib.check(self.lib.ppgpu_children_write(self.h, feas_masks.data_ptr(), survive.data_ptr(), counts.data_ptr(),
                                                     nf, out.data_ptr(), self._stream()), 'children_write')
        return out

    def counters(self, reset: bool = False) -> Dict[str, int]:
        buf = (ctypes.c_uint64 * _lib.NUM_COUNTERS)()
        _lib.check(self.lib.ppgpu_counters(self.h, buf, int(reset), self._stream()), 'counters')
        return {name: int(buf[i]) for i, name in enumerate(_lib.COUNTER_NAMES)}

    def profile(self, on: bool):
        _lib.check(self.lib.ppgpu_profile_enable(self.h, int(on)), 'profile_enable')

    def profile_read(self, reset: bool = False) -> Dict[str, Dict]:
        ms = (ctypes.c_double * _lib.NUM_FAMILIES)()
        ln = (ctypes.c_int64 * _lib.NUM_FAMILIES)()
        _lib.check(self.lib.ppgpu_profile_read(self.h, ms, ln, int(reset)), 'profile_read')
        return {name: dict(ms=float(ms[i]), launches=int(ln[i])) for i, name in enumerate(_lib.FAMILY_NAMES)}

    def launch_count(self) -> int:
        return int(self.lib.ppgpu_launch_count(self.h))

    def masks_from_lists(self, active_sets) -> torch.Tensor:
        out = numpy.zeros((len(active_sets), self.W), dtype=numpy.uint64)
        for ci, aset in enumerate(active_sets):
            for idx in aset:
                i = int(idx) - self.n_eq
                if i >= 0:
                    out[ci, i >> 6] |= numpy.uint64(1) << numpy.uint64(i & 63)
        return torch.from_numpy(out.view(numpy.int64)).to(self.tdev)

    def lists_from_masks(self, masks_np: numpy.ndarray) -> List[List[int]]:
        eq = list(range(self.n_eq))
        m = masks_np.view(numpy.uint64).reshape(-1, self.W)
        bits = numpy.unpackbits(m.view(numpy.uint8).reshape(m.shape[0], -1), axis=1, bitorder='little')
        per_row = bits.sum(1)
        if m.shape[0] and (per_row == per_row[0]).all():
            cols = (numpy.nonzero(bits)[1] + self.n_eq).reshape(m.shape[0], int(per_row[0])).tolist()
            return [eq + c for c in cols] if eq else cols
        return [eq + (numpy.nonzero(r)[0] + self.n_eq).tolist() for r in bits]


def measure_fp64_peak(iters: int = 20000) -> float:
    lib = _lib.load()
    v = ctypes.c_double(0.0)
    _lib.check(lib.ppgpu_measure_fp64_peak(iters, ctypes.byref(v), ctypes.c_void_p(torch.cuda.current_stream().cuda_stream)),
               'fp64 peak')
    return v.value


def _region_classes(program):
    mod = type(program).__module__
    root = mod.split('.mpqp_program')[0].split('.mplp_program')[0]
    if root not in ('ppopt_b200',) and root.endswith('ppopt'):
        import importlib
        try:
            cr = importlib.import_module(root + '.critical_region').CriticalRegion
            sol = importlib.import_module(root + '.solution').Solution
            return cr, sol
        except Exception:
            pass
    from .critical_region import CriticalRegion
    from .solution import Solution
    return CriticalRegion, Solution


def _to_host(x):
    if isinstance(x, torch.Tensor):
        if x.is_cuda:
            h = torch.empty(x.shape, dtype=x.dtype, pin_memory=True)
            h.copy_(x, non_blocking=True)
            torch.cuda.current_stream(x.device).synchronize()
            return h.numpy()
        return x.numpy()
    return numpy.asarray(x)


_INDEX_LISTS_ON_DEVICE = __import__('os').environ.get('PPGPU_ASSEMBLY_DEVICE', '0') == '1'
_PAUSE_GC = __import__('os').environ.get('PPGPU_ASSEMBLY_PAUSE_GC', '0') == '1'


def _kept_index_lists_numpy(kept_all, asets, k_act, n_inact, ne, m):
    ns = kept_all.shape[0]
    ri, ci = numpy.nonzero(kept_all)
    is_l, is_r = ci < k_act, (ci >= k_act) & (ci < k_act + n_inact)
    val = ci - (k_act + n_inact)
    if k_act > 0:
        val = numpy.where(is_l, asets[ri, numpy.minimum(ne + ci, ne + k_act - 1)], val)
    if n_inact > 0:
        act_bool = numpy.zeros((ns, m), dtype=bool)
        if asets.shape[1]:
            act_bool[numpy.arange(ns)[:, None], asets] = True
        inactive = numpy.nonzero(~act_bool)[1].reshape(ns, n_inact)
        val = numpy.where(is_r, inactive[ri, numpy.clip(ci - k_act, 0, n_inact - 1)], val)
    cnt = numpy.stack([kept_all.sum(1), kept_all[:, :k_act].sum(1), kept_all[:, :k_act + n_inact].sum(1)]).astype(numpy.int64)
    return val.astype(numpy.int64), (ci - k_act).astype(numpy.int64), cnt


def _kept_index_lists_torch(kept_all, asets, k_act, n_inact, ne, m):
    ns = kept_all.shape[0]
    nz = torch.nonzero(kept_all)
    ri, ci = nz[:, 0], nz[:, 1]
    val = ci - (k_act + n_inact)
    if k_act > 0:
        val = torch.where(ci < k_act, asets[ri, torch.clamp(ne + ci, max=ne + k_act - 1)], val)
    if n_inact > 0:
        act_bool = torch.zeros((ns, m), dtype=torch.bool, device=kept_all.device)
        if asets.shape[1]:
            act_bool.scatter_(1, asets, True)
        inactive = torch.nonzero(~act_bool)[:, 1].reshape(ns, n_inact)
        is_r = (ci >= k_act) & (ci < k_act + n_inact)
        val = torch.where(is_r, inactive[ri, torch.clamp(ci - k_act, 0, n_inact - 1)], val)
    cnt = torch.stack([kept_all.sum(1), kept_all[:, :k_act].sum(1), kept_all[:, :k_act + n_inact].sum(1)])
    return val, ci - k_act, cnt


def build_regions(eng: Engine, cr_cls, active_sets, k_act, laws, rows, flags, info, d2h: Optional[list] = None) -> list:
    n, t, ne, m = eng.n, eng.t, eng.n_eq, eng.m
    ns = len(active_sets)
    if ns == 0:
        return []
    n_inact = eng.mi - k_act
    on_dev = isinstance(laws, torch.Tensor)
    copied = 0

    def host(x):
        nonlocal copied
        h = _to_host(x.contiguous() if isinstance(x, torch.Tensor) else numpy.ascontiguousarray(x))
        copied += h.nbytes
        return h
    kept_all = (flags & 3) == 3
    nodup_all = kept_all & ((flags & 4) == 0)
    info = host(info)
    emitted = (info[:, 0] == 1.0).tolist()
    A_all, b_all = host(laws[:, :n, 1:]), host(laws[:, :n, :1])
    C_all, d_all = host(laws[:, n:, 1:]), host(laws[:, n:, :1])
    if t != 1:
        E_cat, f_cat = host(rows[:, :, 1:][nodup_all]), host(rows[:, :, :1][nodup_all])
        e_off = numpy.concatenate([[0], numpy.cumsum(host(nodup_all.sum(1)))]).tolist()
    asets = numpy.asarray(active_sets, dtype=numpy.int64).reshape(ns, ne + k_act)
    aset_lists = asets.tolist()
    if on_dev and _INDEX_LISTS_ON_DEVICE:
        val, pos, cnt = _kept_index_lists_torch(kept_all, torch.from_numpy(asets).to(kept_all.device), k_act, n_inact, ne, m)
        val, pos, cnt = host(val), host(pos), host(cnt)
    else:
        val, pos, cnt = _kept_index_lists_numpy(host(kept_all) if on_dev else numpy.asarray(kept_all), asets, k_act, n_inact, ne, m)
    bounds = numpy.concatenate([[0], numpy.cumsum(cnt[0])]).tolist()
    n_l, n_lr = cnt[1].tolist(), cnt[2].tolist()
    val_list, pos_list = val.tolist(), pos.tolist()
    import gc
    gc_was_on = gc.isenabled() and _PAUSE_GC
    if gc_was_on:
        gc.disable()
    try:
        lo_l, hi_l = bounds[:-1], bounds[1:]
        le_l = [lo + x for lo, x in zip(lo_l, n_l)]
        re_l = [lo + x for lo, x in zip(lo_l, n_lr)]
        if t == 1:
            E_l = [numpy.array([[1], [-1]]) for _ in range(ns)]
            f_l = [numpy.array([[hi_], [-lo_]]) for lo_, hi_ in zip(info[:, 2].tolist(), info[:, 3].tolist())]
        else:
            E_l = [E_cat[a:b] for a, b in zip(e_off[:-1], e_off[1:])]
            f_l = [f_cat[a:b] for a, b in zip(e_off[:-1], e_off[1:])]
        out = [cr_cls(A, b, C, d, E, f, aset, val_list[re:hi], val_list[lo:le], [pos_list[le:re], val_list[le:re]]) if em else None
               for A, b, C, d, E, f, aset, lo, le, re, hi, em in zip(list(A_all), list(b_all), list(C_all), list(d_all), E_l, f_l,
                                                                     aset_lists, lo_l, le_l, re_l, hi_l, emitted)]
    finally:
        if gc_was_on:
            gc.enable()
    if d2h is not None:
        d2h.append(copied if on_dev else 0)
    return out


class ParentLevel:
    __slots__ = ('feas_masks', 'ws', 'nf', 'wit')

    def __init__(self, feas_masks, ws, nf, wit):
        self.feas_masks, self.ws, self.nf, self.wit = feas_masks, ws, int(nf), wit


WITNESS_MIN_LEVEL = 100000


def _inherit_on() -> bool:
    import os
    return os.environ.get('PPGPU_INHERIT', '1') != '0'


def _dist():
    import torch.distributed as dist
    if dist.is_available() and dist.is_initialized() and dist.get_world_size() > 1:
        return dist
    return None


class NumericalFailure(RuntimeError):
    """A candidate could not be decided (LP iteration limit / non-finite values) even after the cold re-evaluation.
    Raised instead of silently treating the candidate as infeasible, which would prune every superset of it."""


def _checksum(status: torch.Tensor) -> int:
    n = status.shape[0]
    if n == 0:
        return 0
    w = (torch.arange(n, device=status.device, dtype=torch.int64) * 2654435761 + 12345) & 0x7fffffff
    return int((((status & 15).to(torch.int64) + 1) * w).sum().item() & 0x7fffffffffffffff)


def _eval_level(eng: Engine, masks: torch.Tensor, k_act: int, dist, rank: int, world: int,
                wit: Optional[torch.Tensor] = None, parent: Optional['ParentLevel'] = None) -> torch.Tensor:
    n = masks.shape[0]
    status = torch.zeros((n,), dtype=torch.uint8, device=eng.tdev)
    if world <= 1:
        eng.level_eval(masks, k_act, status, 7, witness=wit, parent=parent)
        return status
    mine = sharding.chunks(n, rank, world)
    if mine:
        if len(mine) == 1:
            lo, hi = mine[0]
            eng.level_eval(masks, k_act, status, 7, lo, hi, witness=wit, parent=parent)
        else:
            packed = torch.cat([masks[lo:hi] for lo, hi in mine])
            wp = torch.zeros((packed.shape[0],) + tuple(wit.shape[1:]), dtype=torch.int64, device=eng.tdev) if wit is not None else None
            st = eng.level_eval(packed, k_act, None, 7, witness=wp, parent=parent)
            off = 0
            for lo, hi in mine:
                status[lo:hi] = st[off:off + hi - lo]
                if wit is not None:
                    wit[lo:hi] = wp[off:off + hi - lo]
                off += hi - lo
    if wit is not None:
        dist.all_reduce(wit, op=dist.ReduceOp.SUM)
    return sharding.gather_status(status, dist)


def _escalate_numeric(eng: Engine, masks: torch.Tensor, status: torch.Tensor, k_act: int, flagged: Dict, level: int):
    num = eng.select(status, ST_NUMERIC | ST_FEAS, ST_NUMERIC)
    if num.shape[0]:
        sub = masks[num].contiguous()
        st2 = torch.full((sub.shape[0],), ST_RANK, dtype=torch.uint8, device=eng.tdev)
        eng.level_eval(sub, k_act, st2, 2 | 4 | 8)
        still = (st2 & (ST_NUMERIC | ST_FEAS)) == ST_NUMERIC
        if bool(still.any().item()):
            bad = eng.lists_from_masks(sub[still][:8].cpu().numpy())
            raise NumericalFailure(f'level {level}: {int(still.sum().item())} candidate(s) undecided after the cold '
                                   f're-evaluation, e.g. {bad}')
        status[num] = st2
        flagged['numeric_recovered'] += int(num.shape[0])
    scr = eng.select(status, ST_NUMERIC | ST_FEAS | ST_OPT, ST_NUMERIC | ST_FEAS)
    if scr.shape[0]:
        status[scr] = (status[scr] & ~ST_NUMERIC) | ST_OPT
        flagged['screen_failed'] += int(scr.shape[0])


def _collect_flags(eng: Engine, masks: torch.Tensor, status: torch.Tensor, flagged: Dict):
    for name, bit in (('border', ST_BORDER), ('thin', ST_THIN)):
        idx = eng.select(status, bit, bit)
        if idx.shape[0]:
            flagged[name + '_count'] += int(idx.shape[0])
            room = 4096 - len(flagged[name])
            if room > 0:
                flagged[name].extend(eng.lists_from_masks(masks[idx[:room]].cpu().numpy()))


def solve(program, max_levels: Optional[int] = None, collect_status: bool = False, engine: Optional[Engine] = None,
          emit_regions: bool = True, distributed: bool = True, expand_last: bool = False,
          materialize: bool = True, digest: bool = False):
    own = engine is None
    eng = Engine(program_arrays(program)) if own else engine
    cr_cls, sol_cls = _region_classes(program)
    dist = _dist() if distributed else None
    rank, world = (dist.get_rank(), dist.get_world_size()) if dist is not None else (0, 1)
    regions: list = []
    stats = []
    statuses = []
    sums = []
    flagged = {'border': [], 'thin': [], 'border_count': 0, 'thin_count': 0, 'numeric_recovered': 0, 'screen_failed': 0,
               'singular_skipped': []}
    depth = eng.max_depth if max_levels is None else min(eng.max_depth, max_levels)
    complete = max_levels is None or max_levels >= eng.max_depth
    masks = eng.root_level() if depth > 0 else eng.empty((0, eng.W), torch.int64)
    total = 0
    inherit = _inherit_on() and eng.has_walk_vertex
    parent = None
    for lvl in range(depth):
        n = masks.shape[0]
        if n == 0:
            break
        t0 = time.perf_counter()
        k_act = lvl + 1
        last = lvl + 1 == eng.max_depth or (lvl + 1 == depth and not expand_last)
        wit = torch.zeros((n, _lib.WITNESS_SLOTS, eng.W), dtype=torch.int64, device=eng.tdev) \
            if (inherit and not last and n >= WITNESS_MIN_LEVEL) else None
        status = _eval_level(eng, masks, k_act, dist, rank, world, wit, parent)
        parent = None
        any_flag = int((status & (ST_NUMERIC | ST_THIN | ST_BORDER)).max().item()) if n else 0
        if any_flag & ST_NUMERIC:
            _escalate_numeric(eng, masks, status, k_act, flagged, lvl + 1)
        n_reg = 0
        opt_idx = eng.select(status, ST_OPT, ST_OPT)
        n_opt = int(opt_idx.shape[0])
        if n_opt and emit_regions:
            mine = sharding.owned(opt_idx, n, rank, world) if world > 1 else opt_idx
            if not materialize:
                if mine.shape[0]:
                    eng.emit(masks, mine, k_act, status)
                if world > 1 and (digest or collect_status):
                    status = sharding.gather_region_bits(status, mine, dist)
            else:
                bufs = eng.emit(masks, mine, k_act, status) if mine.shape[0] else None
                if world > 1:
                    mine, bufs = sharding.gather_regions(eng, mine, bufs, k_act, dist)
                    status = sharding.gather_region_bits(status, mine, dist, already_global=True, bufs=bufs)
                if bufs is not None and mine.shape[0]:
                    laws, rows, flags, info = bufs
                    sel_masks = masks[mine].cpu().numpy()
                    eng.d2h_bytes += sel_masks.nbytes
                    asets = eng.lists_from_masks(sel_masks)
                    sing = torch.nonzero(info[:, 0] < 0).reshape(-1).cpu().numpy()
                    if sing.size:
                        if eng.use_gram or not eng.is_qp:
                            raise numpy.linalg.LinAlgError('Singular matrix')
                        flagged['singular_skipped'].extend(asets[i] for i in sing[:256])
                    copied = []
                    built = build_regions(eng, cr_cls, asets, k_act, laws, rows, flags, info, d2h=copied)
                    eng.d2h_bytes += sum(copied)
                    regions.extend(r for r in built if r is not None)
            after = torch.stack([((status & ST_REGION) != 0).sum(), (status & (ST_THIN | ST_BORDER)).max().to(torch.int64)]).cpu()
            n_reg = int(after[0])
            any_flag |= int(after[1])
        if last:
            feas_idx = None
            n_feas = int(((status & ST_FEAS) != 0).sum().item())
        else:
            feas_idx = eng.select(status, ST_FEAS, ST_FEAS)
            n_feas = int(feas_idx.shape[0])
        if any_flag & (ST_THIN | ST_BORDER):
            _collect_flags(eng, masks, status, flagged)
        if collect_status:
            statuses.append((masks.cpu().numpy(), status.cpu().numpy()))
        if digest:
            sums.append((n, _checksum(status)))
        keep = {} if wit is not None else None
        nxt = eng.children(masks, feas_idx, k_act, dist if world > 1 else None, keep) if not last else eng.empty((0, eng.W), torch.int64)
        if keep:
            parent = ParentLevel(keep['feas_masks'], keep['ws'], keep['nf'], wit[feas_idx].contiguous())
        torch.cuda.synchronize(eng.tdev)
        total += n
        stats.append(dict(level=lvl + 1, candidates=n, feasible=n_feas, optimal=n_opt, regions=n_reg,
                          seconds=time.perf_counter() - t0))
        masks = nxt
    frontier = int(masks.shape[0])
    base_status = 0
    if complete:
        m0 = torch.zeros((1, eng.W), dtype=torch.int64, device=eng.tdev)
        st0 = eng.level_eval(m0, 0)
        sel0 = eng.select(st0, ST_OPT, ST_OPT)
        if sel0.shape[0] and emit_regions:
            laws, rows, flags, info = [x.cpu().numpy() for x in eng.emit(m0, sel0, 0, st0)]
            if info[0, 0] < 0:
                raise numpy.linalg.LinAlgError('Singular matrix')
            reg = build_regions(eng, cr_cls, [list(range(eng.n_eq))], 0, laws, rows, flags, info)[0]
            if reg is not None and info[0, 1] > 1e-8:
                regions.append(reg)
        base_status = int(st0.cpu().numpy()[0])
    solution = sol_cls(program, regions)
    solution.level_stats = stats
    solution.total_candidates = total
    solution.frontier = frontier
    solution.base_status = base_status
    solution.engine_counters = eng.counters()
    solution.gpu_launches = eng.launch_count()
    solution.h2d_bytes, solution.d2h_bytes = eng.h2d_bytes, eng.d2h_bytes
    solution.flagged = flagged
    if collect_status:
        solution.level_status = statuses
    if digest:
        import hashlib
        hh = hashlib.sha256(repr(sums).encode())
        if materialize:
            hh.update(repr([tuple(r.active_set) for r in regions]).encode())
        solution.digest = hh.hexdigest()
    if own:
        eng.close()
    return solution
```

Measured before the change: 341.1 million.

## Replace per-set hash lookups with prefix-group index for children counting and inheritance

Builds a grouped index over lexicographically sorted feasible parents, keyed by each set's prefix without its last element, with a bitmask of the last elements present. Children counting now runs one thread per parent and intersects group bitmasks across the parent's subsets, instead of a warp testing each candidate child with separate hash probes per subset. Inheritance uses the same group index, and the kernels are templated on word count. It adds several extra kernel launches, a lexicographic-order check with an additional host readback, and depends on the parents arriving sorted.

```diff
diff --git a/include/ppgpu.h b/include/ppgpu.h
--- a/include/ppgpu.h
+++ b/include/ppgpu.h
@@ -56,6 +56,7 @@
                        const void* d_parent_ws, const uint64_t* d_parent_wit, ppgpu_stream stream);
 
 size_t ppgpu_scan_workspace_bytes(int64_t n);
+size_t ppgpu_select_workspace_bytes(int64_t n);
 int ppgpu_level_select(ppgpu_program* prog, const uint8_t* d_status, int64_t n, uint8_t bits, uint8_t value,
                        int64_t* d_idx_out, int64_t* h_count, void* d_ws, size_t ws_bytes, ppgpu_stream stream);
 
diff --git a/ppopt_b200/_lib.py b/ppopt_b200/_lib.py
--- a/ppopt_b200/_lib.py
+++ b/ppopt_b200/_lib.py
@@ -37,6 +37,7 @@
     'ppgpu_level_eval': (ctypes.c_int, [_vp, _vp, _i64, _i32, _vp, _i32, _vp]),
     'ppgpu_level_eval_w': (ctypes.c_int, [_vp, _vp, _i64, _i32, _vp, _i32, _vp, _vp, _i64, _vp, _vp, _vp]),
     'ppgpu_scan_workspace_bytes': (_sz, [_i64]),
+    'ppgpu_select_workspace_bytes': (_sz, [_i64]),
     'ppgpu_level_select': (ctypes.c_int, [_vp, _vp, _i64, _u8, _u8, _vp, ctypes.POINTER(_i64), _vp, _sz, _vp]),
     'ppgpu_regions_emit': (ctypes.c_int, [_vp, _vp, _vp, _i64, _i32, _vp, _vp, _vp, _vp, _vp, _vp]),
     'ppgpu_children_count': (ctypes.c_int, [_vp, _vp, _vp, _i64, _i32, _vp, _vp, _vp, ctypes.POINTER(_i64), _vp, _sz, _vp]),
diff --git a/ppopt_b200/csrc/api.cu b/ppopt_b200/csrc/api.cu
--- a/ppopt_b200/csrc/api.cu
+++ b/ppopt_b200/csrc/api.cu
@@ -363,6 +363,7 @@
 }
 
 size_t ppgpu_scan_workspace_bytes(int64_t n) { return scan_workspace_bytes(n); }
+size_t ppgpu_select_workspace_bytes(int64_t n) { return select_workspace_bytes(n); }
 
 int ppgpu_level_select(ppgpu_program* p, const uint8_t* d_status, int64_t n, uint8_t bits, uint8_t value,
                        int64_t* d_idx_out, int64_t* h_count, void* d_ws, size_t ws_bytes, ppgpu_stream stream) {
@@ -370,8 +371,8 @@
     *h_count = 0;
     if (n <= 0) return 0;
     cudaStream_t st = (cudaStream_t)stream;
-    if (ws_bytes < scan_workspace_bytes(n)) return fail_msg("workspace too small");
-    long long* d_count = (long long*)d_ws + (scan_workspace_bytes(n) / sizeof(long long) - 1);
+    if (ws_bytes < select_workspace_bytes(n)) return fail_msg("workspace too small");
+    long long* d_count = (long long*)d_ws + (select_workspace_bytes(n) / sizeof(long long) - 1);
     cudaError_t e;
     {
         ProfScope ps(p, st, 6);
@@ -417,11 +418,13 @@
                            (long long*)d_offsets, d_ws, ws_bytes, p->d_counters, st);
     }
     if (e != cudaSuccess) return fail("K6 count", e);
-    p->launches += 5;
-    long long tot = 0;
+    p->launches += 12;
+    long long tot = 0, disorder = 0;
     e = cudaMemcpyAsync(&tot, (long long*)d_offsets + nf, sizeof(long long), cudaMemcpyDeviceToHost, st);
+    if (e == cudaSuccess) e = cudaMemcpyAsync(&disorder, children_order_flag(d_ws, nf), sizeof(long long), cudaMemcpyDeviceToHost, st);
     if (e == cudaSuccess) e = cudaStreamSynchronize(st);
     if (e != cudaSuccess) return fail("K6 total", e);
+    if (disorder) return fail_msg("K6: the feasible parents are not one level's sets in lexicographic order");
     *h_total = tot;
     return 0;
 }
@@ -436,7 +439,7 @@
         e = children_prepare(p->dev, d_masks, (const long long*)d_feas_idx, nf, d_feas_masks, d_ws, ws_bytes, (cudaStream_t)stream);
     }
     if (e != cudaSuccess) return fail("K6 prepare", e);
-    p->launches += 3;
+    p->launches += 8;
     return 0;
 }
 
@@ -472,10 +475,12 @@
     }
     if (e != cudaSuccess) return fail("K6 scan", e);
     p->launches += 2;
-    long long tot = 0;
+    long long tot = 0, disorder = 0;
     e = cudaMemcpyAsync(&tot, (long long*)d_counts_to_offsets + nf, sizeof(long long), cudaMemcpyDeviceToHost, st);
+    if (e == cudaSuccess) e = cudaMemcpyAsync(&disorder, children_order_flag(d_ws, nf), sizeof(long long), cudaMemcpyDeviceToHost, st);
     if (e == cudaSuccess) e = cudaStreamSynchronize(st);
     if (e != cudaSuccess) return fail("K6 total", e);
+    if (disorder) return fail_msg("K6: the feasible parents are not one level's sets in lexicographic order");
     *h_total = tot;
     return 0;
 }
diff --git a/ppopt_b200/csrc/k6_children.cu b/ppopt_b200/csrc/k6_children.cu
--- a/ppopt_b200/csrc/k6_children.cu
+++ b/ppopt_b200/csrc/k6_children.cu
@@ -6,6 +6,9 @@
 constexpr int SCAN_THREADS = 256;
 constexpr int SCAN_ITEMS = 8;
 constexpr int SCAN_CHUNK = SCAN_THREADS * SCAN_ITEMS;
+constexpr int MAXW = 4;
+
+static long long table_words(long long nf) { return 2 * nf + 2 > 512 ? 2 * nf + 2 : 512; }
 
 __device__ __forceinline__ long long block_exclusive_scan(long long v, long long* total) {
     __shared__ long long wsum[SCAN_THREADS / 32];
@@ -85,10 +88,8 @@
 }
 
 
-size_t scan_workspace_bytes(long long n) {
-    const long long nb = (n + SCAN_CHUNK - 1) / SCAN_CHUNK + 1;
-    const long long table = 2 * n + 2 > 1024 ? 2 * n + 2 : 1024;
-    return (size_t)(n + 1 + nb + 2 + table) * sizeof(long long);
+size_t select_workspace_bytes(long long n) {
+    return (size_t)(n + 1 + (n + SCAN_CHUNK - 1) / SCAN_CHUNK + 3) * sizeof(long long);
 }
 
 static cudaError_t scan_inplace(long long* vals, long long n, long long* bsum, cudaStream_t st) {
@@ -114,7 +115,7 @@
 
 cudaError_t select_indices(const uint8_t* status, long long n, uint8_t bits, uint8_t value, long long* idx_out,
                            long long* d_count, void* ws, size_t ws_bytes, cudaStream_t st) {
-    if (ws_bytes + sizeof(long long) < (size_t)(n + 1 + (n + SCAN_CHUNK - 1) / SCAN_CHUNK + 3) * sizeof(long long)) return cudaErrorInvalidValue;
+    if (ws_bytes + sizeof(long long) < select_workspace_bytes(n)) return cudaErrorInvalidValue;
     long long* offs = (long long*)ws;
     long long* bsum = offs + n + 1;
     if (n == 0) return cudaMemsetAsync(d_count, 0, sizeof(long long), st);
@@ -147,8 +148,6 @@
     return cudaGetLastError();
 }
 
-constexpr int MAXW = 4;
-
 __global__ void gather_masks_kernel(const uint64_t* __restrict__ masks, const long long* __restrict__ idx, long long nf, int W,
                                     uint64_t* __restrict__ out) {
     const long long e = (long long)blockIdx.x * blockDim.x + threadIdx.x;
@@ -185,95 +184,202 @@
     return (unsigned)h;
 }
 
-__global__ void hash_insert_kernel(const uint64_t* __restrict__ feas, long long nf, int W, int* __restrict__ table, unsigned cap_mask) {
+__device__ __forceinline__ Mask4 load_mask(const uint64_t* __restrict__ m, long long i, int W) {
+    Mask4 k;
+#pragma unroll
+    for (int x = 0; x < MAXW; ++x) k.w[x] = x < W ? __ldg(m + i * W + x) : 0ull;
+    return k;
+}
+
+__device__ __forceinline__ bool mask_eq(const Mask4& a, const Mask4& b) {
+    bool eq = true;
+#pragma unroll
+    for (int x = 0; x < MAXW; ++x) eq &= a.w[x] == b.w[x];
+    return eq;
+}
+
+__device__ __forceinline__ int pop_last(Mask4& k) {
+    int last = -1;
+#pragma unroll
+    for (int x = MAXW - 1; x >= 0; --x)
+        if (last < 0 && k.w[x]) {
+            const int b = 63 - __clzll((long long)k.w[x]);
+            k.w[x] &= ~(1ull << b);
+            last = x * 64 + b;
+        }
+    return last;
+}
+
+__device__ __forceinline__ uint64_t low_bits(int b) { return b <= 0 ? 0ull : b >= 64 ? ~0ull : (1ull << b) - 1ull; }
+
+__device__ __forceinline__ Mask4 row_range(int lo, int hi) {
+    Mask4 r;
+#pragma unroll
+    for (int x = 0; x < MAXW; ++x) r.w[x] = low_bits(hi - 64 * x) & ~low_bits(lo - 64 * x);
+    return r;
+}
+
+struct GroupIndex {
+    long long* hdr;
+    int* table;
+    uint64_t* rec;
+};
+
+static GroupIndex group_index(void* ws, long long nf) {
+    long long* base = (long long*)ws + (nf + SCAN_CHUNK - 1) / SCAN_CHUNK + 2;
+    GroupIndex gi;
+    gi.hdr = base;
+    gi.table = reinterpret_cast<int*>(base + 4);
+    gi.rec = reinterpret_cast<uint64_t*>(base + 4 + table_words(nf));
+    return gi;
+}
+
+static size_t group_index_bytes(long long nf, int W) {
+    const long long nb = (nf + SCAN_CHUNK - 1) / SCAN_CHUNK;
+    return (size_t)(nb + 6 + table_words(nf) + (long long)(W + 1) * nf) * sizeof(long long);
+}
+
+size_t scan_workspace_bytes(long long n) { return group_index_bytes(n, MAXW); }
+
+const long long* children_order_flag(const void* ws, long long nf) { return group_index(const_cast<void*>(ws), nf).hdr + 2; }
+
+__global__ void group_flag_kernel(const uint64_t* __restrict__ feas, long long nf, int W, long long* __restrict__ flag,
+                                  GroupIndex gi) {
     const long long p = (long long)blockIdx.x * blockDim.x + threadIdx.x;
     if (p >= nf) return;
-    Mask4 k;
-#pragma unroll
-    for (int x = 0; x < MAXW; ++x) k.w[x] = x < W ? feas[p * W + x] : 0ull;
-    unsigned slot = hash_mask(k, W) & cap_mask;
-    while (atomicCAS(&table[slot], -1, (int)p) != -1) slot = (slot + 1) & cap_mask;
-}
-
-__device__ __forceinline__ bool hash_contains(const uint64_t* __restrict__ feas, int W, const int* __restrict__ table,
-                                              unsigned cap_mask, const Mask4& key) {
-    unsigned slot = hash_mask(key, W) & cap_mask;
+    const Mask4 m = load_mask(feas, p, W);
+    Mask4 q = m;
+    pop_last(q);
+    bool first = p == 0;
+    if (!first) {
+        const Mask4 prev = load_mask(feas, p - 1, W);
+        int cp = 0, cm = 0;
+#pragma unroll
+        for (int x = 0; x < MAXW; ++x) { cp += __popcll(prev.w[x]); cm += __popcll(m.w[x]); }
+        if (cp != cm || lex_cmp4(feas + (p - 1) * W, m, W) >= 0) gi.hdr[2] = 1;
+        Mask4 r = prev;
+        pop_last(r);
+        first = !mask_eq(q, r);
+    }
+    flag[p] = first ? 1 : 0;
+}
+
+__global__ void group_build_kernel(const uint64_t* __restrict__ feas, long long nf, int W, const long long* __restrict__ gid,
+                                   GroupIndex gi) {
+    const long long p = (long long)blockIdx.x * blockDim.x + threadIdx.x;
+    if (p >= nf) return;
+    if (p == 0) {
+        const long long groups = gid[nf];
+        long long cap = 1024;
+        while (cap < 2 * groups) cap <<= 1;
+        gi.hdr[0] = cap - 1;
+        gi.hdr[1] = groups;
+    }
+    const long long g = gid[p];
+    if (gid[p + 1] == g) return;
+    Mask4 q = load_mask(feas, p, W);
+    Mask4 e = row_range(0, 0);
+    int last = pop_last(q);
+    for (long long r = p + 1;; ++r) {
+        const Mask4 bit = row_range(last, last + 1);
+#pragma unroll
+        for (int x = 0; x < MAXW; ++x) e.w[x] |= bit.w[x];
+        if (r >= nf) break;
+        Mask4 s = load_mask(feas, r, W);
+        last = pop_last(s);
+        if (!mask_eq(s, q)) break;
+    }
+    uint64_t* r = gi.rec + g * (W + 1);
+    r[0] = (uint64_t)p;
+#pragma unroll
+    for (int x = 0; x < MAXW; ++x)
+        if (x < W) r[1 + x] = e.w[x];
+}
+
+__global__ void group_clear_kernel(GroupIndex gi) {
+    const long long s = (long long)blockIdx.x * blockDim.x + threadIdx.x;
+    if (s <= gi.hdr[0]) gi.table[s] = -1;
+}
+
+__global__ void group_insert_kernel(const uint64_t* __restrict__ feas, int W, GroupIndex gi) {
+    const long long g = (long long)blockIdx.x * blockDim.x + threadIdx.x;
+    if (g >= gi.hdr[1]) return;
+    const unsigned cap_mask = (unsigned)gi.hdr[0];
+    Mask4 q = load_mask(feas, (long long)gi.rec[g * (W + 1)], W);
+    pop_last(q);
+    unsigned slot = hash_mask(q, W) & cap_mask;
+    while (atomicCAS(&gi.table[slot], -1, (int)g) != -1) slot = (slot + 1) & cap_mask;
+}
+
+__device__ __forceinline__ bool find_group(const uint64_t* __restrict__ feas, int W, const GroupIndex& gi, unsigned cap_mask,
+                                           const Mask4& q, Mask4& e) {
+    unsigned slot = hash_mask(q, W) & cap_mask;
     for (;;) {
-        const int e = __ldg(table + slot);
-        if (e < 0) return false;
-        bool same = true;
-#pragma unroll
-        for (int x = 0; x < MAXW; ++x)
-            if (x < W && feas[(long long)e * W + x] != key.w[x]) same = false;
-        if (same) return true;
+        const int g = __ldg(gi.table + slot);
+        if (g < 0) return false;
+        const uint64_t* r = gi.rec + (long long)g * (W + 1);
+        e = load_mask(r + 1, 0, W);
+        Mask4 k = load_mask(feas, (long long)__ldg(r), W);
+        pop_last(k);
+        if (mask_eq(k, q)) return true;
         slot = (slot + 1) & cap_mask;
     }
 }
 
-__global__ void __launch_bounds__(128)
+template <int W>
+__global__ void __launch_bounds__(256, 3)
 children_count_kernel(DevProgram P, const uint64_t* __restrict__ feas, long long p_lo, long long p_hi, int k_act,
                       uint64_t* __restrict__ survive, long long* __restrict__ counts,
-                      unsigned long long* __restrict__ counters, const int* __restrict__ table, unsigned cap_mask) {
-    const int lane = threadIdx.x & 31;
-    const long long warp0 = ((long long)blockIdx.x * blockDim.x + threadIdx.x) >> 5;
-    const long long nwarps = ((long long)gridDim.x * blockDim.x) >> 5;
-    const int W = P.W, mi = P.mi;
-    const bool lp = !P.is_qp;
-    const int child_limit = lp ? (P.ne + k_act + 1) + P.m - P.n : 0x7fffffff;
-    const int sub_limit = lp ? (P.ne + k_act) + P.m - P.n : 0x7fffffff;
+                      unsigned long long* __restrict__ counters, GroupIndex gi) {
+    const long long p = p_lo + (long long)blockIdx.x * blockDim.x + threadIdx.x;
     unsigned long long lookups = 0;
-    for (long long p = p_lo + warp0; p < p_hi; p += nwarps) {
-        uint64_t pm[MAXW];
-#pragma unroll
-        for (int w = 0; w < MAXW; ++w) pm[w] = w < W ? feas[p * W + w] : 0ull;
-        int last = -1;
-#pragma unroll
-        for (int w = MAXW - 1; w >= 0; --w)
-            if (last < 0 && pm[w]) last = w * 64 + 63 - __clzll((long long)pm[w]);
+    if (p < p_hi) {
+        const unsigned cap_mask = (unsigned)__ldg(gi.hdr);
+        const bool lp = !P.is_qp;
+        const long long child_limit = lp ? (long long)(P.ne + k_act + 1) + P.m - P.n : (long long)P.ne + P.mi;
+        const long long sub_limit = lp ? child_limit - 1 : (long long)P.ne + P.mi;
+        const Mask4 pm = load_mask(feas, p, W);
+        Mask4 rest = pm;
+        const int last = pop_last(rest);
+        const int hi = (int)(child_limit - P.ne < P.mi ? child_limit - P.ne : P.mi);
+        const int wlo = (int)(sub_limit - P.ne > last + 1 ? sub_limit - P.ne : last + 1);
+        const Mask4 range = row_range(last + 1, hi), waived = row_range(wlo, hi);
+        Mask4 acc;
+#pragma unroll
+        for (int x = 0; x < MAXW; ++x) acc.w[x] = x < W ? ~0ull : 0ull;
+        bool open = true;
+#pragma unroll
+        for (int w = MAXW - 1; w >= 0; --w) {
+            uint64_t bits = pm.w[w];
+            while (bits && open) {
+                uint64_t left = 0;
+#pragma unroll
+                for (int x = 0; x < MAXW; ++x) left |= range.w[x] & ~waived.w[x] & acc.w[x];
+                open = left != 0;
+                if (!open) break;
+                const int b = 63 - __clzll((long long)bits);
+                bits &= ~(1ull << b);
+                Mask4 q = pm;
+                q.w[w] &= ~(1ull << b);
+                ++lookups;
+                Mask4 e;
+                const bool found = find_group(feas, W, gi, cap_mask, q, e);
+#pragma unroll
+                for (int x = 0; x < MAXW; ++x) acc.w[x] &= found ? e.w[x] : 0ull;
+            }
+        }
         long long cnt = 0;
-        uint64_t sv[MAXW];
-#pragma unroll
-        for (int w = 0; w < MAXW; ++w) sv[w] = 0ull;
-        for (int base = ((last + 1) >> 5) << 5; base < mi; base += 32) {
-            const int i = base + lane;
-            bool ok = i > last && i < mi && (P.ne + i) < child_limit;
-            if (ok) {
-                const bool sub_filtered = (P.ne + i) >= sub_limit;
-                if (!sub_filtered) {
-                    Mask4 child;
-#pragma unroll
-                    for (int w = 0; w < MAXW; ++w) child.w[w] = pm[w] | ((w == (i >> 6)) ? (1ull << (i & 63)) : 0ull);
-#pragma unroll
-                    for (int w = 0; w < MAXW; ++w) {
-                        if (w < W) {
-                            uint64_t bits = pm[w];
-                            while (bits && ok) {
-                                const int b = __ffsll((long long)bits) - 1;
-                                bits &= bits - 1;
-                                Mask4 sub;
-#pragma unroll
-                                for (int x = 0; x < MAXW; ++x) sub.w[x] = child.w[x] & ~((x == w) ? (1ull << b) : 0ull);
-                                ++lookups;
-                                if (!hash_contains(feas, W, table, cap_mask, sub)) ok = false;
-                            }
-                        }
-                    }
-                }
-            }
-            const unsigned bal = __ballot_sync(0xffffffffu, ok);
-            cnt += __popc(bal);
-#pragma unroll
-            for (int w = 0; w < MAXW; ++w)
-                if (w == (base >> 6)) sv[w] |= (uint64_t)bal << (base & 63);
+#pragma unroll
+        for (int x = 0; x < MAXW; ++x) {
+            const uint64_t sv = range.w[x] & (waived.w[x] | acc.w[x]);
+            cnt += __popcll(sv);
+            if (x < W) survive[p * W + x] = sv;
         }
-        if (lane == 0) {
-            counts[p] = cnt;
-            for (int w = 0; w < W; ++w) survive[p * W + w] = sv[w];
-        }
+        counts[p] = cnt;
     }
 #pragma unroll
     for (int o = 16; o > 0; o >>= 1) lookups += __shfl_xor_sync(0xffffffffu, lookups, o);
-    if (lane == 0 && lookups) atomicAdd(&counters[CNT_K6_LOOKUPS], lookups);
+    if ((threadIdx.x & 31) == 0 && lookups) atomicAdd(&counters[CNT_K6_LOOKUPS], lookups);
 }
 
 __global__ void __launch_bounds__(128)
@@ -297,26 +403,27 @@
     }
 }
 
-static unsigned hash_capacity(long long nf) {
-    unsigned cap = 1024;
-    while ((long long)cap < 2 * nf) cap <<= 1;
-    return cap;
-}
-
 cudaError_t children_prepare(const DevProgram& P, const uint64_t* masks, const long long* feas_idx, long long nf,
                              uint64_t* feas_masks, void* ws, size_t ws_bytes, cudaStream_t st) {
     if (P.W > MAXW) return cudaErrorInvalidValue;
     if (nf <= 0) return cudaSuccess;
     if (nf >= (1ll << 30)) return cudaErrorInvalidValue;
-    const long long nb = (nf + SCAN_CHUNK - 1) / SCAN_CHUNK;
-    const unsigned cap = hash_capacity(nf);
-    if (ws_bytes < (size_t)(nb + 2) * sizeof(long long) + (size_t)cap * sizeof(int)) return cudaErrorInvalidValue;
-    int* table = reinterpret_cast<int*>((long long*)ws + nb + 2);
+    if (ws_bytes < group_index_bytes(nf, P.W)) return cudaErrorInvalidValue;
+    const GroupIndex gi = group_index(ws, nf);
+    long long* gid = reinterpret_cast<long long*>(gi.table);
     const long long ne = nf * P.W;
+    const unsigned blocks = (unsigned)((nf + 255) / 256);
     gather_masks_kernel<<<(unsigned)((ne + 255) / 256), 256, 0, st>>>(masks, feas_idx, nf, P.W, feas_masks);
-    cudaError_t e = cudaMemsetAsync(table, 0xff, (size_t)cap * sizeof(int), st);
+    cudaError_t e = cudaMemsetAsync(gi.hdr, 0, 4 * sizeof(long long), st);
     if (e != cudaSuccess) return e;
-    hash_insert_kernel<<<(unsigned)((nf + 255) / 256), 256, 0, st>>>(feas_masks, nf, P.W, table, cap - 1);
+    group_flag_kernel<<<blocks, 256, 0, st>>>(feas_masks, nf, P.W, gid, gi);
+    e = scan_inplace(gid, nf, (long long*)ws, st);
+    if (e != cudaSuccess) return e;
+    group_build_kernel<<<blocks, 256, 0, st>>>(feas_masks, nf, P.W, gid, gi);
+    long long cap = 1024;
+    while (cap < 2 * nf) cap <<= 1;
+    group_clear_kernel<<<(unsigned)(cap / 256), 256, 0, st>>>(gi);
+    group_insert_kernel<<<blocks, 256, 0, st>>>(feas_masks, P.W, gi);
     return cudaGetLastError();
 }
 
@@ -324,13 +431,15 @@
                                  long long* counts, long long p_lo, long long p_hi, void* ws, unsigned long long* counters,
                                  cudaStream_t st) {
     if (p_hi <= p_lo) return cudaSuccess;
-    const long long nb = (nf + SCAN_CHUNK - 1) / SCAN_CHUNK;
-    const unsigned cap = hash_capacity(nf);
-    const int* table = reinterpret_cast<const int*>((long long*)ws + nb + 2);
-    long long blocks = ((p_hi - p_lo) * 32 + 127) / 128;
-    if (blocks > 148 * 64) blocks = 148 * 64;
-    children_count_kernel<<<(unsigned)blocks, 128, 0, st>>>(P, feas_masks, p_lo, p_hi, k_act, survive, counts, counters, table,
-                                                            cap - 1);
+    const unsigned blocks = (unsigned)((p_hi - p_lo + 255) / 256);
+    const GroupIndex gi = group_index(ws, nf);
+    switch (P.W) {
+        case 1: children_count_kernel<1><<<blocks, 256, 0, st>>>(P, feas_masks, p_lo, p_hi, k_act, survive, counts, counters, gi); break;
+        case 2: children_count_kernel<2><<<blocks, 256, 0, st>>>(P, feas_masks, p_lo, p_hi, k_act, survive, counts, counters, gi); break;
+        case 3: children_count_kernel<3><<<blocks, 256, 0, st>>>(P, feas_masks, p_lo, p_hi, k_act, survive, counts, counters, gi); break;
+        case 4: children_count_kernel<4><<<blocks, 256, 0, st>>>(P, feas_masks, p_lo, p_hi, k_act, survive, counts, counters, gi); break;
+        default: return cudaErrorInvalidValue;
+    }
     return cudaGetLastError();
 }
 
@@ -358,34 +467,19 @@
     return cudaGetLastError();
 }
 
-__device__ __forceinline__ int hash_find(const uint64_t* __restrict__ feas, int W, const int* __restrict__ table,
-                                         unsigned cap_mask, const Mask4& key) {
-    unsigned slot = hash_mask(key, W) & cap_mask;
-    for (;;) {
-        const int e = __ldg(table + slot);
-        if (e < 0) return -1;
-        bool same = true;
-#pragma unroll
-        for (int x = 0; x < MAXW; ++x)
-            if (x < W && feas[(long long)e * W + x] != key.w[x]) same = false;
-        if (same) return e;
-        slot = (slot + 1) & cap_mask;
-    }
-}
-
+template <int W>
 __global__ void __launch_bounds__(256)
-inherit_kernel(int W, const uint64_t* __restrict__ masks, long long n, uint8_t* __restrict__ status,
-               uint64_t* __restrict__ witness_out, const uint64_t* __restrict__ pfeas, const int* __restrict__ table,
-               unsigned cap_mask, const uint64_t* __restrict__ pwit, unsigned long long* __restrict__ counters) {
+inherit_kernel(const uint64_t* __restrict__ masks, long long n, uint8_t* __restrict__ status,
+               uint64_t* __restrict__ witness_out, const uint64_t* __restrict__ pfeas, GroupIndex gi,
+               const uint64_t* __restrict__ pwit, unsigned long long* __restrict__ counters) {
     const long long i = (long long)blockIdx.x * blockDim.x + threadIdx.x;
     unsigned long long lookups = 0;
     int got = 0;
     if (i < n) {
         const uint8_t sb = status[i];
         if ((sb & PPG_ST_RANK) && !(sb & PPG_ST_FEAS)) {
-            Mask4 m;
-#pragma unroll
-            for (int x = 0; x < MAXW; ++x) m.w[x] = x < W ? masks[i * W + x] : 0ull;
+            const unsigned cap_mask = (unsigned)__ldg(gi.hdr);
+            const Mask4 m = load_mask(masks, i, W);
 #pragma unroll
             for (int w = MAXW - 1; w >= 0; --w) {
                 if (w < W && !got) {
@@ -393,31 +487,52 @@
                     while (bits && !got) {
                         const int b = 63 - __clzll((long long)bits);
                         bits &= ~(1ull << b);
-                        Mask4 sub = m;
-#pragma unroll
-                        for (int x = 0; x < MAXW; ++x)
-                            if (x == w) sub.w[x] &= ~(1ull << b);
+                        Mask4 q = m;
+                        q.w[w] &= ~(1ull << b);
+                        const Mask4 sub = q;
+                        const int h = pop_last(q);
+                        if (h < 0) continue;
                         ++lookups;
-                        const int e = hash_find(pfeas, W, table, cap_mask, sub);
-                        if (e < 0) continue;
-#pragma unroll
-                        for (int sl = 0; sl < PPG_WITNESS_SLOTS; ++sl) {
-                            if (got) continue;
-                            bool inside = true;
-                            uint64_t wv[MAXW];
+                        const Mask4 below = row_range(0, h), bit = row_range(h, h + 1);
+                        unsigned slot = hash_mask(q, W) & cap_mask;
+                        for (;;) {
+                            const int g = __ldg(gi.table + slot);
+                            if (g < 0) break;
+                            slot = (slot + 1) & cap_mask;
+                            const uint64_t* r = gi.rec + (long long)g * (W + 1);
+                            const Mask4 eq = load_mask(r + 1, 0, W);
+                            long long e = (long long)__ldg(r);
+                            uint64_t in = 0;
 #pragma unroll
                             for (int x = 0; x < MAXW; ++x) {
-                                wv[x] = x < W ? __ldg(pwit + ((long long)e * PPG_WITNESS_SLOTS + sl) * W + x) : 0ull;
-                                if (m.w[x] & ~wv[x]) inside = false;
+                                e += __popcll(eq.w[x] & below.w[x]);
+                                in |= eq.w[x] & bit.w[x];
                             }
-                            if (inside) {
-                                got = 1;
-                                status[i] = sb | PPG_ST_FEAS;
-                                if (witness_out)
-#pragma unroll
-                                    for (int x = 0; x < MAXW; ++x)
-                                        if (x < W) witness_out[i * (PPG_WITNESS_SLOTS * W) + x] = wv[x];
+                            if (!in) continue;
+                            const Mask4 pm = load_mask(pfeas, e, W);
+                            uint64_t wv[PPG_WITNESS_SLOTS][MAXW];
+#pragma unroll
+                            for (int sl = 0; sl < PPG_WITNESS_SLOTS; ++sl)
+#pragma unroll
+                                for (int x = 0; x < MAXW; ++x)
+                                    wv[sl][x] = x < W ? __ldg(pwit + ((e * PPG_WITNESS_SLOTS + sl) * W + x)) : 0ull;
+                            if (!mask_eq(pm, sub)) continue;
+#pragma unroll
+                            for (int sl = 0; sl < PPG_WITNESS_SLOTS; ++sl) {
+                                bool inside = !got;
+#pragma unroll
+                                for (int x = 0; x < MAXW; ++x)
+                                    if (m.w[x] & ~wv[sl][x]) inside = false;
+                                if (inside) {
+                                    got = 1;
+                                    status[i] = sb | PPG_ST_FEAS;
+                                    if (witness_out)
+#pragma unroll
+                                        for (int x = 0; x < MAXW; ++x)
+                                            if (x < W) witness_out[i * (PPG_WITNESS_SLOTS * W) + x] = wv[sl][x];
+                                }
                             }
+                            break;
                         }
                     }
                 }
@@ -438,11 +553,15 @@
                            unsigned long long* counters, cudaStream_t st) {
     if (n <= 0 || parent_nf <= 0) return cudaSuccess;
     if (P.W > MAXW) return cudaErrorInvalidValue;
-    const long long nb = (parent_nf + SCAN_CHUNK - 1) / SCAN_CHUNK;
-    const unsigned cap = hash_capacity(parent_nf);
-    const int* table = reinterpret_cast<const int*>((const long long*)parent_ws + nb + 2);
-    inherit_kernel<<<(unsigned)((n + 255) / 256), 256, 0, st>>>(P.W, masks, n, status, witness_out, parent_feas, table, cap - 1,
-                                                                parent_wit, counters);
+    const GroupIndex gi = group_index(const_cast<void*>(parent_ws), parent_nf);
+    const unsigned blocks = (unsigned)((n + 255) / 256);
+    switch (P.W) {
+        case 1: inherit_kernel<1><<<blocks, 256, 0, st>>>(masks, n, status, witness_out, parent_feas, gi, parent_wit, counters); break;
+        case 2: inherit_kernel<2><<<blocks, 256, 0, st>>>(masks, n, status, witness_out, parent_feas, gi, parent_wit, counters); break;
+        case 3: inherit_kernel<3><<<blocks, 256, 0, st>>>(masks, n, status, witness_out, parent_feas, gi, parent_wit, counters); break;
+        case 4: inherit_kernel<4><<<blocks, 256, 0, st>>>(masks, n, status, witness_out, parent_feas, gi, parent_wit, counters); break;
+        default: return cudaErrorInvalidValue;
+    }
     return cudaGetLastError();
 }
 
diff --git a/ppopt_b200/csrc/launch.h b/ppopt_b200/csrc/launch.h
--- a/ppopt_b200/csrc/launch.h
+++ b/ppopt_b200/csrc/launch.h
@@ -55,6 +55,8 @@
                       unsigned long long* counters, int sm_count, cudaStream_t st);
 
 size_t scan_workspace_bytes(long long n);
+size_t select_workspace_bytes(long long n);
+const long long* children_order_flag(const void* ws, long long nf);
 cudaError_t select_indices(const uint8_t* status, long long n, uint8_t bits, uint8_t value, long long* idx_out,
                            long long* d_count, void* ws, size_t ws_bytes, cudaStream_t st);
 cudaError_t root_level(const DevProgram& P, uint64_t* masks, long long* d_count, cudaStream_t st);
diff --git a/ppopt_b200/engine.py b/ppopt_b200/engine.py
--- a/ppopt_b200/engine.py
+++ b/ppopt_b200/engine.py
@@ -114,7 +114,7 @@
         n = status.shape[0]
         if n == 0:
             return self.empty((0,), torch.int64)
-        ws_bytes = self.lib.ppgpu_scan_workspace_bytes(n)
+        ws_bytes = self.lib.ppgpu_select_workspace_bytes(n)
         ws = self.empty(((ws_bytes + 7) // 8,), torch.int64)
         idx = self.empty((n,), torch.int64)
         cnt = ctypes.c_int64(0)
```

After: 357.4 million (median of 6 runs). 1.05x the previous value.
